# tardis-sn/tardis

Measured on AMD Instinct MI355X. Metric: packets/sec, higher is better.
Workload: dtype f64; 1 GPU; BASELINE configs[2]: 100000000 packets/GPU/step, 20 shells, 500000 lines, macroatom, 0 v-packets, last-interaction tracking on; synthetic opacities (SURVEY 8d, heavy-tailed macro-atom blocks), packets from the device black-body source (T_inner = 10000 K); level_sizes=heavy, packets_per_gpu=100000000, n_shells=20, n_lines=500000, line_interaction_type=macroatom, n_vpackets=0, parallelism=single GPU

## Files before the change

include/tardis_mc.h:

```cpp
#ifndef TARDIS_MC_H
#define TARDIS_MC_H

#include <stdint.h>

#ifdef __cplusplus
extern "C" {
#endif

#define TARDIS_MC_ABI_VERSION 2

enum {
    TARDIS_MC_OK = 0,
    TARDIS_MC_ERR_INVALID_ARGUMENT = -1,
    TARDIS_MC_ERR_HIP = -2,
    TARDIS_MC_ERR_MONTECARLO = -3,
    TARDIS_MC_ERR_MACRO_ATOM = -4,
    TARDIS_MC_ERR_UNSUPPORTED = -5,
    TARDIS_MC_ERR_COMM = -6,
    TARDIS_MC_ERR_STATE = -7
};

enum { TARDIS_MC_LINE_SCATTER = 0, TARDIS_MC_LINE_DOWNBRANCH = 1, TARDIS_MC_LINE_MACROATOM = 2 };

typedef struct TardisMcConfig {
// ... 83 lines not shown
    int64_t dropped;
    int64_t *offsets;
    int64_t *event_id, *interaction_type, *status, *shell_id, *after_shell_id, *line_absorb_id, *line_emit_id;
    double *radius, *before_nu, *before_mu, *before_energy, *after_nu, *after_mu, *after_energy;
} TardisMcEventLog;

typedef struct TardisMcDecomposition {
    int64_t n_classes;
    const int64_t *line_class;
    double time_of_simulation;
    double nu_start, nu_end;
    double *emission;
    double *absorption;
    double *no_interaction;
    double *electron_scatter;
    int64_t *shell_packets;
    int64_t *line_emit_packets;
    int64_t *line_absorb_packets;
    int64_t n_selected, n_line, n_electron_scatter, n_no_interaction;
} TardisMcDecomposition;

typedef struct TardisMcVpacketLog {
    int64_t capacity;
    int64_t count;
    int64_t *offsets;
    int64_t *source_packet;
    double *nus, *energies, *initial_mus, *initial_rs;
    double *last_interaction_in_nu, *last_interaction_in_r;
    int64_t *last_interaction_type, *last_interaction_in_id, *last_interaction_out_id, *last_interaction_shell_id;
} TardisMcVpacketLog;

typedef struct TardisMcContext TardisMcContext;

int tardis_mc_abi_version(void);
int tardis_mc_device_count(void);
int tardis_mc_create(int device_id, TardisMcContext **out_ctx);
void tardis_mc_destroy(TardisMcContext *ctx);
const char *tardis_mc_last_error(const TardisMcContext *ctx);

int tardis_mc_set_option(TardisMcContext *ctx, const char *name, long long value);

int tardis_mc_set_geometry(TardisMcContext *ctx, const TardisMcGeometry *geometry);
int tardis_mc_set_opacity(TardisMcContext *ctx, const TardisMcOpacity *opacity);
int tardis_mc_set_config(TardisMcContext *ctx, const TardisMcConfig *config);
int tardis_mc_set_packets(TardisMcContext *ctx, const TardisMcPackets *packets);
int tardis_mc_reset_estimators(TardisMcContext *ctx);
int tardis_mc_propagate(TardisMcContext *ctx);
int tardis_mc_synchronize(TardisMcContext *ctx);
int tardis_mc_last_propagate_ms(TardisMcContext *ctx, double *out_ms);
int tardis_mc_last_kernel_times(TardisMcContext *ctx, double *out_seed_ms, double *out_propagate_ms, int *out_launches);
int tardis_mc_last_estimator_ms(TardisMcContext *ctx, double *out_ms);
int tardis_mc_last_counters(TardisMcContext *ctx, int64_t out_counters[TARDIS_MC_N_COUNTERS]);
int tardis_mc_last_variant(TardisMcContext *ctx);
int tardis_mc_last_table_offsets(TardisMcContext *ctx);
int tardis_mc_last_compactions(TardisMcContext *ctx);
int tardis_mc_last_tracker_defer(TardisMcContext *ctx);
int tardis_mc_kernel_table_row(int table, int row, int key[12]);
int tardis_mc_last_kernel_key(TardisMcContext *ctx, int *table, int key[12]);
int tardis_mc_progress(TardisMcContext *ctx, int64_t *out_packets_started, int64_t *out_packets_total);
int tardis_mc_get_results(TardisMcContext *ctx, TardisMcResult *result);

int tardis_mc_pcg64_seed(uint64_t seed, uint64_t out_state[4]);
int tardis_mc_create_blackbody_packets(TardisMcContext *ctx, int64_t n_total, int64_t first, int64_t count, double radius,
                                       double temperature, const uint64_t pcg_state[4], uint32_t max_seed_val,
                                       const double *l_array, int64_t n_l);
int tardis_mc_get_packets(TardisMcContext *ctx, double *initial_radii, double *initial_nus, double *initial_mus,
                          double *initial_energies, int64_t *packet_seeds);

int tardis_mc_packet_spectrum(TardisMcContext *ctx, double time_of_simulation, double luminosity_nu_start,
                              double luminosity_nu_end, double *emitted_luminosity_hist, double *reabsorbed_luminosity_hist,
                              double *out_emitted_luminosity, double *out_reabsorbed_luminosity);

int tardis_mc_packet_decomposition(TardisMcContext *ctx, TardisMcDecomposition *d);
int tardis_mc_vpacket_decomposition(TardisMcContext *ctx, TardisMcDecomposition *d);
int tardis_mc_decomposition_path(int64_t n_classes, int64_t n_bins, int64_t n_shells);

int tardis_mc_radiation_field(TardisMcContext *ctx, double time_of_simulation, const double *volume, double w_epsilon,
                              int detailed_optical_window, double *t_radiative, double *dilution_factor, double *j_blues);

int tardis_mc_formal_integral(TardisMcContext *ctx, double inner_temperature, const double *frequencies, int64_t n_frequencies,
                              const double *att_S_ul, const double *Jred_lu, const double *Jblue_lu, int64_t n_impact_parameters,
                              double *luminosity_densities, double *intensities_nu_p);

int tardis_mc_source_function(TardisMcContext *ctx, double time_of_simulation, const double *volume, const double *wavelength_cm,
                              double *att_S_ul, double *Jred_lu, double *Jblue_lu, double *e_dot_u);
int tardis_mc_last_source_iterations(TardisMcContext *ctx);
int tardis_mc_formal_integral_resident(TardisMcContext *ctx, double inner_temperature, const double *frequencies, int64_t n_frequencies,
                                       int64_t n_impact_parameters, double *luminosity_densities, double *intensities_nu_p);

int tardis_mc_formal_integral_interpolated(TardisMcContext *ctx, int64_t interpolate_shells, double inner_temperature,
                                           const double *frequencies, int64_t n_frequencies, int64_t n_impact_parameters,
                                           double *luminosity_densities, double *intensities_nu_p);
int tardis_mc_interpolated_source(TardisMcContext *ctx, int64_t interpolate_shells, double *r_inner_i, double *r_outer_i,
                                  double *electron_density_i, double *tau_sobolev_i, double *att_S_ul_i, double *Jred_lu_i,
                                  double *Jblue_lu_i, double *e_dot_u_i);

typedef struct TardisMcLineData {
    int64_t n_lines;
    int64_t n_transitions;
    int64_t n_levels;
    const double *f_lu;
    const double *wavelength_cm;
    const double *g_lower;
    const double *g_upper;
    const int64_t *level_lower;
    const int64_t *level_upper;
// ... 141 lines not shown
```

tardis_amd/_lib.py:

```python
from __future__ import annotations

import ctypes as C
import os
import subprocess

from . import _abi

_HERE = os.path.dirname(os.path.abspath(__file__))
LIB_PATH = os.environ.get("TARDIS_MC_LIB") or os.path.join(_HERE, "libtardis_mc_hip.so")
_lib = None

_vp, _i, _ll = C.c_void_p, C.c_int, C.c_longlong
SYMBOLS = {
    "tardis_mc_abi_version": (_i, []),
    "tardis_mc_device_count": (_i, []),
    "tardis_mc_create": (_i, [_i, C.POINTER(_vp)]),
    "tardis_mc_destroy": (None, [_vp]),
    "tardis_mc_last_error": (C.c_char_p, [_vp]),
    "tardis_mc_set_option": (_i, [_vp, C.c_char_p, _ll]),
    "tardis_mc_set_geometry": (_i, [_vp, _vp]),
    "tardis_mc_set_opacity": (_i, [_vp, _vp]),
    "tardis_mc_set_config": (_i, [_vp, _vp]),
    "tardis_mc_set_packets": (_i, [_vp, _vp]),
    "tardis_mc_reset_estimators": (_i, [_vp]),
    "tardis_mc_propagate": (_i, [_vp]),
    "tardis_mc_synchronize": (_i, [_vp]),
    "tardis_mc_last_propagate_ms": (_i, [_vp, C.POINTER(C.c_double)]),
    "tardis_mc_last_kernel_times": (_i, [_vp, C.POINTER(C.c_double), C.POINTER(C.c_double), C.POINTER(C.c_int)]),
    "tardis_mc_last_estimator_ms": (_i, [_vp, C.POINTER(C.c_double)]),
    "tardis_mc_last_counters": (_i, [_vp, C.POINTER(C.c_int64)]),
    "tardis_mc_last_variant": (_i, [_vp]),
    "tardis_mc_last_table_offsets": (_i, [_vp]),
    "tardis_mc_last_compactions": (_i, [_vp]),
    "tardis_mc_last_tracker_defer": (_i, [_vp]),
    "tardis_mc_kernel_table_row": (_i, [_i, _i, C.POINTER(_i)]),
    "tardis_mc_last_kernel_key": (_i, [_vp, C.POINTER(_i), C.POINTER(_i)]),
    "tardis_mc_progress": (_i, [_vp, C.POINTER(C.c_int64), C.POINTER(C.c_int64)]),
    "tardis_mc_get_results": (_i, [_vp, _vp]),
    "tardis_mc_pcg64_seed": (_i, [C.c_uint64, C.POINTER(C.c_uint64)]),
    "tardis_mc_create_blackbody_packets": (_i, [_vp, C.c_int64, C.c_int64, C.c_int64, C.c_double, C.c_double,
                                                C.POINTER(C.c_uint64), C.c_uint32, _vp, C.c_int64]),
    "tardis_mc_get_packets": (_i, [_vp] * 6),
    "tardis_mc_packet_spectrum": (_i, [_vp, C.c_double, C.c_double, C.c_double, _vp, _vp, C.POINTER(C.c_double), C.POINTER(C.c_double)]),
    "tardis_mc_packet_decomposition": (_i, [_vp, _vp]),
    "tardis_mc_vpacket_decomposition": (_i, [_vp, _vp]),
    "tardis_mc_decomposition_path": (_i, [C.c_int64, C.c_int64, C.c_int64]),
    "tardis_mc_radiation_field": (_i, [_vp, C.c_double, _vp, C.c_double, C.c_int, _vp, _vp, _vp]),
    "tardis_mc_formal_integral": (_i, [_vp, C.c_double, _vp, C.c_int64, _vp, _vp, _vp, C.c_int64, _vp, _vp]),
    "tardis_mc_source_function": (_i, [_vp, C.c_double, _vp, _vp, _vp, _vp, _vp, _vp]),
    "tardis_mc_last_source_iterations": (_i, [_vp]),
    "tardis_mc_formal_integral_resident": (_i, [_vp, C.c_double, _vp, C.c_int64, C.c_int64, _vp, _vp]),
    "tardis_mc_formal_integral_interpolated": (_i, [_vp, C.c_int64, C.c_double, _vp, C.c_int64, C.c_int64, _vp, _vp]),
    "tardis_mc_interpolated_source": (_i, [_vp, C.c_int64] + [_vp] * 8),
    "tardis_mc_set_line_data": (_i, [_vp, _vp]),
    "tardis_mc_update_opacity": (_i, [_vp, _vp]),
    "tardis_mc_get_opacity": (_i, [_vp] * 6),
    "tardis_mc_last_opacity_update_ms": (_i, [_vp] + [C.POINTER(C.c_double)] * 3),
    "tardis_mc_opacity_update_path": (_i, [C.c_int64]),
    "tardis_mc_set_plasma_data": (_i, [_vp, _vp]),
    "tardis_mc_update_plasma": (_i, [_vp, _vp]),
    "tardis_mc_get_plasma": (_i, [_vp] * 5 + [C.POINTER(C.c_int32)]),
    "tardis_mc_last_plasma_update_ms": (_i, [_vp] + [C.POINTER(C.c_double)] * 4),
    "tardis_mc_plasma_update_path": (_i, [C.c_int64]),
    "tardis_mc_set_ionization_options": (_i, [_vp, _vp]),
    "tardis_mc_check_ionization_options": (_i, [_vp, C.c_int64, _vp, _vp, _vp]),
    "tardis_mc_get_helium": (_i, [_vp, _vp, _vp]),
    "tardis_mc_last_helium_ms": (_i, [_vp, C.POINTER(C.c_double)]),
    "tardis_mc_set_nlte_data": (_i, [_vp, _vp]),
    "tardis_mc_check_nlte_data": (_i, [_vp, C.c_int64, _vp, C.c_int64, _vp, _vp]),
    "tardis_mc_get_nlte": (_i, [_vp, _vp, _vp]),
    "tardis_mc_last_nlte_ms": (_i, [_vp] + [C.POINTER(C.c_double)] * 2),
    "tardis_mc_nlte_solve_path": (_i, [C.c_int64]),
    "tardis_mc_nlte_solve_form": (_i, [C.c_int64]),
    "tardis_mc_set_nlte_collision_data": (_i, [_vp, _vp]),
    "tardis_mc_check_nlte_collision_data": (_i, [_vp, C.c_int64, _vp, C.c_double, C.c_int64, _vp]),
    "tardis_mc_get_nlte_collision_rates": (_i, [_vp, _vp, _vp]),
    "tardis_mc_get_event_log": (_i, [_vp, _vp]),
    "tardis_mc_get_vpacket_log": (_i, [_vp, _vp]),
    "tardis_mc_stream_results": (_i, [_vp, _vp]),
    "tardis_mc_streamed_packets": (_i, [_vp, C.POINTER(C.c_int64), C.POINTER(C.c_int64)]),
    "tardis_mc_run": (_i, [_vp] * 6),
    "tardis_mc_comm_get_unique_id": (_i, [_vp]),
    "tardis_mc_comm_init": (_i, [_vp, _i, _i, _vp]),
    "tardis_mc_allreduce_estimators": (_i, [_vp]),
# ... 40 lines not shown
```

tardis_amd/csrc/propagate_plan.hpp:

```cpp
#pragma once

#include "../../include/tardis_mc.h"

namespace plan {

constexpr int DBG_WALK_LANE_FP64 = 128;
constexpr int DBG_WALK_GROUP_FP64 = 8192;
constexpr int DBG_LONG_INSTANTIATIONS = 1048576;
constexpr int DBG_NO_SCREENING = 33554432;
constexpr int DBG_WAVE_COUNTERS = 1 | 2 | 4 | 16 | 32 | 16384 | 32768 | 65536 | 131072 | 524288 | 2097152 | 4194304 | 8388608 | 16777216 | 134217728 | 268435456;
constexpr int DBG_FP64_WALKS = DBG_WALK_LANE_FP64 | DBG_WALK_GROUP_FP64;
constexpr int DBG_WAVE_CROSS_CHECK = DBG_FP64_WALKS | DBG_LONG_INSTANTIATIONS | DBG_WAVE_COUNTERS;

struct PlanInput {
    int n_shells, n_lines, n_trans;
    long long n_packets;
    long long number_of_vpackets;
    double survival_probability;
    int enable_full_relativity, line_interaction_type;
    bool lines_sorted, prob_negative, have_walk_tables;
    int variant, table_offsets, vpacket_screening;
    long long vpk_wave_min_packets;
    bool track_full;
    int debug_flags;
    bool pfx_valid, pfx_negative;
};

struct Plan {
    int variant;
    bool cooperative;
    bool w64;
    bool screen_on;
    int last_variant, last_table_offsets;
    int error;
    const char *message;
};

inline Plan plan_error(Plan p, const char *message)
{
    p.error = TARDIS_MC_ERR_INVALID_ARGUMENT;
    p.message = message;
    return p;
}

inline Plan plan_propagate(const PlanInput &in)
{
    Plan p{};
    p.error = TARDIS_MC_OK;
    p.message = "";
    const bool vpk = in.number_of_vpackets > 0;
    const bool small_shape = in.n_shells <= 30 && in.n_lines <= 100000;
    const bool screen_auto = (long long)in.n_lines >= 2500LL * (long long)in.n_shells;
    const bool screen = in.vpacket_screening < 0 ? screen_auto : in.vpacket_screening != 0;
    p.screen_on = vpk && in.survival_probability == 0.0 && screen && !(in.debug_flags & DBG_NO_SCREENING) && !(in.pfx_valid && in.pfx_negative);
    const bool prefer_lane_sweeps = !in.enable_full_relativity && !vpk;
    const bool vpk_wave = vpk && (small_shape || (p.screen_on && in.n_packets >= in.vpk_wave_min_packets));
    const int wave_auto = prefer_lane_sweeps ? 3 : 2;
    int variant = in.variant >= 0 ? in.variant : ((vpk && in.number_of_vpackets > 32) ? 0 : (vpk ? (vpk_wave ? 2 : 1) : wave_auto));
    auto is_wave = [](int v) { return v == 2 || v == 3 || v == 4; };
    if (in.prob_negative && (variant == 2 || variant == 3)) variant = 1;
    if (vpk && in.survival_probability > 0.0 && is_wave(variant)) variant = 1;
    if (variant == 4 && !vpk) variant = wave_auto;
    if (in.prob_negative && variant == 4) variant = 1;
    if (in.track_full) {
        const bool wave_ok = in.lines_sorted && !in.prob_negative && !(vpk && (in.number_of_vpackets > 32 || in.survival_probability > 0.0)) &&
                             (in.line_interaction_type == 0 || in.have_walk_tables) && !(in.debug_flags & DBG_WAVE_CROSS_CHECK) && in.n_packets < (1LL << 31);
        variant = (wave_ok && variant != 0) ? 2 : 0;
    }
    bool cooperative = in.lines_sorted && (variant == 1 || is_wave(variant)) && (!vpk || in.number_of_vpackets <= 32);
    const bool big_tables = (long long)in.n_shells * in.n_lines >= (1LL << 28) || (long long)in.n_shells * in.n_trans >= (1LL << 28);
    bool w64 = false;
    if (cooperative && (in.table_offsets == 1 || (in.table_offsets < 0 && big_tables))) {
        if (variant == 4)
            return plan_error(p, "variant 4 (the volley queue) has no 64-bit table offsets: n_shells * n_lines or n_shells * n_trans "
                                 "reaches 2^28, or option table_offsets is 1; use the automatic variant");
        if (is_wave(variant) && (in.debug_flags & DBG_WAVE_CROSS_CHECK))
            return plan_error(p, "the cross-check instantiations of the wave kernel (debug flags 128, 8192, 1048576 and the counter "
                                 "flags) have no 64-bit table offsets");
        if (is_wave(variant) && (long long)in.n_shells * in.n_lines >= (1LL << 32)) {
            if (in.variant >= 0)
                return plan_error(p, "n_shells * n_lines reaches 2^32: the line-visit log of the wave kernels (variants 2-4) "
                                     "indexes (shell, line) in 32 bits; use variant 1 or the automatic variant");
            if (in.track_full) { cooperative = false; variant = 0; }
            else { variant = 1; w64 = true; }
        } else if (is_wave(variant) && in.line_interaction_type != 0 && !in.have_walk_tables) {
            cooperative = false;
            variant = 0;
        } else
            w64 = true;
    }
    if (cooperative && big_tables && !w64)
        return plan_error(p, "n_shells * n_lines or n_shells * n_trans reaches 2^28, the limit of the cooperative kernels' 32-bit "
                             "table offsets, and option table_offsets is 0");
    p.variant = variant;
    p.cooperative = cooperative;
    p.w64 = w64;
    p.last_table_offsets = (w64 || !cooperative) ? 64 : 32;
    p.last_variant = cooperative ? ((variant == 3 && in.enable_full_relativity) ? 2 : variant) : 0;
    if (!cooperative) p.screen_on = false;
    return p;
}

}
```

tardis_amd/csrc/propagate_wave.hpp:

```cpp
#pragma once
#include "mc_device.hpp"
#include "propagate_group.hpp"
#include "estimator_log.hpp"
#include "walk_tables.hpp"
#include "event_log.hpp"
#include "mt_generation.hpp"

namespace mc {

constexpr int WV_STATE_STRIDE = 624;
constexpr int WV_RING = 8, WV_RING_VPK = 16;
enum : int { WS_NEED_PACKET = 0, WS_NEED_TRACE = 1, WS_SWEEP = 2, WS_DONE = 3, WS_WALK = 4, WS_VOLLEY = 5, WS_VCARRY = 6 };
constexpr int RES_PENDING = -1;
constexpr int WV_DBG_FLAGS = 1 | 2 | 4 | 16 | 32 | 16384 | 32768 | 65536 | 131072 | 524288 | 2097152 | 4194304 | 8388608 | 16777216 | 134217728 | 268435456;
constexpr int WV_RESERVE = 32;

struct WaveShared {
    double nu[64], rcp_nu[64], comov_nu[64], chi[64], rcp_chi[64], tau_event[64], d_cont0[64];
    double d_boundary[64];
    int res_info[64], res_line[64];
    unsigned rng_a[64], rng_b[64];
    int cursor[64], rowfast[64];
    int queue[64];
};
constexpr size_t WAVE_SHARED_LS_BYTES = sizeof(WaveShared) - 3 * 64 * sizeof(int);
static_assert(offsetof(WaveShared, queue) + sizeof(int) * 64 == sizeof(WaveShared) && offsetof(WaveShared, cursor) + 3 * 64 * sizeof(int) == sizeof(WaveShared),
              "cursor | rowfast | queue are the last 768 bytes: the lane-sweep instantiations leave them out, the pooled volleys' item list lies over them");
struct WaveSharedFull {
    double r[64], mu[64];
};

template <bool FULL, bool VPK, bool LS = false, bool SL = false>
__host__ __device__ constexpr size_t wave_kernel_lds_bytes(int n_shells)
{
    return (LS ? WAVE_SHARED_LS_BYTES : sizeof(WaveShared)) + (FULL ? sizeof(WaveSharedFull) : 0) + (size_t)(VPK ? WV_RING_VPK : WV_RING) * 64 * sizeof(double) +
           (size_t)(VPK ? 6 : 5) * (size_t)n_shells * sizeof(double) +
           (SL ? (size_t)n_shells * 2 * sizeof(unsigned) : 0);
}

struct __attribute__((aligned(16))) VpResult {
    double nu, energy, mu0;
    int used, visits, err, pad;
};
struct __attribute__((aligned(16))) VpPark {
    double r, mu, nu, energy, tau, mu0, rcp_nu, margin, v0_r, v0_energy;
    int shell, next_line, owner, item, q, used, avail, head, v0_shell, v0_line;
    unsigned visits;
    int flags;
};
constexpr int VP_ROUND = 6;
static_assert(2 * VP_ROUND + 3 <= 16, "a round's mu and roulette draws, plus the 4 doubles of the refill that completes them, must fit WV_RING_VPK");

struct __attribute__((aligned(16))) VolleyRequest {
    double r, mu, nu, energy;
    int shell, next_line, vdone, cnt;
    unsigned pred_bits;
    int pad0, pad1, pad2;
    double draws[WV_RING_VPK];
};
// ... 5 lines not shown
    double t_exp;
    const int2 *line_block;
    int ls_min_active, ls_max_steps;
    int walk_min_active;
    int vq_min_active;
};
struct LaunchRec;
struct __attribute__((aligned(16))) LaneSave {
    double r, mu, nu, energy, dop;
    double s_tau, s_tau_event, s_kp, s_xb;
    double d_cont0, d_boundary;
    double ring[WV_RING_VPK];
    int shell, next_line, status, state, pkt, pflags, r_gpos, r_head, r_cnt;
    int trk_count, trk_boundary, flags;
    int s_line;
    unsigned s_row;
    int res_info, res_line, pre_blk_x, pre_blk_y;
    unsigned rng_a, rng_b;
    int vseq;
    unsigned pred_bits;
    int vdone, pad_v0, pad_v1, pad_v2;
    double walk_inv_new, walk_block, trk_nu, trk_mu, trk_energy;
    double walk_event, pad_w;
};
struct WaveSave {
    long long res_next, res_end;
    int exhausted, done;
    int log_chunk, log_gen;
    unsigned long long cnt[7];
};
struct WaveCold {
    GroupArgs P;
    DeviceProblem D;
    EstimatorLog log;
    uint32_t *seeded_states;
    long long chunk_first, chunk_count;
    const LaunchRec *launch;
    VpResult *vp_scratch;
    VpPark *vp_park;
    int vp_carry_min_active;
    int trk_defer;
    LaneSave *save;
    WaveSave *wsave;
    int resume;
    int drain_split;
    unsigned *suspended;
    VolleyRequest *vq_req;
    unsigned *vq_items;
    unsigned *vq_count;
    int log_continue;
    int log_gen;
    double *vq_jsave;
    int rng_complete;
};

__global__ void __launch_bounds__(64) late_list_kernel(const LaneSave *__restrict__ save, const WaveSave *__restrict__ wsave, int waves, long long first, long long end,
                                                       unsigned *__restrict__ late, unsigned *__restrict__ late_count, unsigned capacity)
{
    const int w = blockIdx.x, lane = threadIdx.x;
    if (w >= waves) return;
    const WaveSave ws = wsave[w];
    if (ws.done) return;
    const LaneSave &v = save[(size_t)w * 64 + lane];
    const bool live = v.state != WS_NEED_PACKET && v.state != WS_DONE && (long long)v.pkt >= first && (long long)v.pkt < end;
    const long long r0 = ws.res_next > first ? ws.res_next : first, r1 = ws.res_end < end ? ws.res_end : end;
    const int n_res = r1 > r0 ? (int)(r1 - r0) : 0;
    const unsigned long long lm = __ballot(live);
    const unsigned n_live = (unsigned)__popcll(lm);
    unsigned base = 0;
    if (lane == 0 && n_live + (unsigned)n_res > 0) base = atomicAdd(late_count, n_live + (unsigned)n_res);
    base = (unsigned)__shfl((int)base, 0);
    if (live) {
        const unsigned pos = base + (unsigned)__popcll(lm & ((1ull << lane) - 1ull));
        if (pos < capacity) late[pos] = (unsigned)v.pkt;
    }
    for (int k = lane; k < n_res; k += 64) {
        const unsigned pos = base + n_live + (unsigned)k;
        if (pos < capacity) late[pos] = (unsigned)(r0 + k);
    }
}

__global__ void __launch_bounds__(64) drain_census_kernel(const LaneSave *__restrict__ save, const WaveSave *__restrict__ wsave, int waves, long long n_packets,
                                                          unsigned *__restrict__ out)
{
    const int w = blockIdx.x, lane = threadIdx.x;
    if (w >= waves) return;
    const WaveSave ws = wsave[w];
    if (ws.done) return;
    const int state = save[(size_t)w * 64 + lane].state;
    const unsigned n_live = (unsigned)__popcll(__ballot(state != WS_NEED_PACKET && state != WS_DONE));
    const unsigned n_need = (unsigned)__popcll(__ballot(state == WS_NEED_PACKET));
    const long long r1 = ws.res_end < n_packets ? ws.res_end : n_packets;
    if (lane == 0) {
        if (n_live) atomicAdd(out, n_live);
        if (r1 > ws.res_next) atomicAdd(out + 1, (unsigned)(r1 - ws.res_next));
        atomicAdd(out + 2, 1u);
        if (n_need) atomicAdd(out + 3, n_need);
    }
}
__global__ void __launch_bounds__(64) drain_compact_kernel(const LaneSave *__restrict__ save, const WaveSave *__restrict__ wsave, const uint32_t *__restrict__ states, int waves,
                                                           LaneSave *__restrict__ dst_save, uint32_t *__restrict__ dst_states, unsigned *__restrict__ counter, unsigned density)
{
    const int w = blockIdx.x, lane = threadIdx.x;
    if (w >= waves) return;
    const WaveSave ws = wsave[w];
    if (ws.done) return;
// ... 90 lines not shown
            }
            s.owner = -1;
        } else {
            const int n_in = min(G, L - s.cur0);
            visits += (unsigned long long)n_in;
            s.tau_carry = gbcast<G>(tau_incl, n_in - 1);
            s.d_cont_carry = exact_div<FAST>(s.tau_event - s.tau_carry, s.chi, s.rcp_chi);
            s.cur0 += G;
            s.nu_line = nu_next;
            s.tau_line = tau_next;
        }
    } else {
        if (j == 0) {
            const bool cont = s.d_cont_carry < s.d_boundary;
            sh.d_boundary[s.owner] = cont ? s.d_cont_carry : s.d_boundary;
            sh.res_line[s.owner] = 0;
            sh.res_info[s.owner] = (cont ? 2 : 1) | 8;
        }
        s.owner = -1;
    }
}


__device__ __forceinline__ int lane_exact_line(const WaveHot &P, int line, double nu_line, double tau_line, double tau_prev, double nu,
                                               double comov_nu, double chi, double tau_event, double d_boundary, double &distance)
{
    const double tau_incl = tau_prev + tau_line;
    const double d_cont = (tau_event - tau_prev) / chi;
    const bool is_last = line == P.n_lines - 1;
    const double nu_diff = comov_nu - nu_line;
    const double q = nu_diff / nu;
    const bool close = fabs(q) < CLOSE_LINE_THRESHOLD;
    const bool err = !is_last && !close && !(nu_diff >= 0);
    const double d_far = q * C_LIGHT * P.t_exp;
    const double d_trace = is_last ? MISS_DISTANCE : (close ? 0.0 : d_far);
    const double tau_combined = tau_incl + chi * d_trace;
    double dmin = d_trace;
    if (d_boundary < dmin) dmin = d_boundary;
    if (d_cont < dmin) dmin = d_cont;
    const bool stop_b = !err && d_trace != 0 && dmin == d_boundary;
    const bool stop_e = !err && d_trace != 0 && !stop_b && dmin == d_cont;
    const bool stop_l = !err && !stop_b && !stop_e && tau_combined > tau_event && !P.disable_line_scattering;
    distance = stop_b ? d_boundary : (stop_e ? d_cont : d_trace);
    return stop_b ? 1 : (stop_e ? 2 : (stop_l ? 3 : (err ? 4 : 0)));
}
constexpr int LS_CHUNK = 8;
#ifndef TMC_STRAIGHT_A
#define TMC_STRAIGHT_A 0
#endif
#ifndef TMC_LS_CHUNK_NT
#define TMC_LS_CHUNK_NT 10
#endif
constexpr int LS_CHUNK_NT = TMC_LS_CHUNK_NT;

__global__ void __launch_bounds__(256) macro_cumulative_kernel(const double *__restrict__ prob_t, double *__restrict__ cum_t,
                                                                const int *__restrict__ block_edge, int n_blocks, long long n_trans,
                                                                int n_shells, int *negative)
{
    const long long i = (long long)blockIdx.x * blockDim.x + threadIdx.x;
    if (i >= (long long)n_blocks * n_shells) return;
    const int b = (int)(i % n_blocks), s = (int)(i / n_blocks);
    const double *p = prob_t + (long long)s * n_trans;
    double *c = cum_t + (long long)s * n_trans;
    double carry = 0.0;
    bool neg = false;
    const int b0 = block_edge[b], b1 = block_edge[b + 1];
    for (int k0 = b0; k0 < b1; k0 += 8) {
        double v[8];
#pragma unroll
        for (int q = 0; q < 8; ++q) v[q] = k0 + q < b1 ? p[k0 + q] : 0.0;
#pragma unroll
        for (int q = 0; q < 8; ++q)
            if (k0 + q < b1) {
                neg |= !(v[q] >= 0.0);
                carry += v[q];
                c[k0 + q] = carry;
            }
    }
    if (neg) atomicOr(negative, 1);
}

struct __attribute__((aligned(16))) TrackerRecord {
    double before_nu, before_mu, before_energy, radius, after_mu;
    int shell, type, absorb, emit, count, valid;
};
static_assert(sizeof(TrackerRecord) == 64, "TrackerRecord is one 64-byte request");

__global__ void __launch_bounds__(256) tracker_unpack_kernel(DeviceProblem D, long long first, long long count, const unsigned *__restrict__ index = nullptr)
{
    const long long j = (long long)blockIdx.x * blockDim.x + threadIdx.x;
    if (j >= count) return;
    const long long i = index ? (long long)index[j] : first + j;
    const double e = D.out_e[i];
    if (e == -99.0) return;
    const TrackerRecord r = reinterpret_cast<const TrackerRecord *>(D.li_rec)[i];
    const bool any = r.valid != 0 && r.count > 0;
    const double nan = __builtin_nan("");
    const double nu = D.out_nu[i], en = fabs(e);
    D.li_radius[i] = any ? r.radius : nan;
    D.li_nu[i] = any ? nu : nan; D.li_energy[i] = any ? en : nan;
    D.li_before_nu[i] = any ? r.before_nu : nan; D.li_before_mu[i] = any ? r.before_mu : nan; D.li_before_energy[i] = any ? r.before_energy : nan;
    D.li_after_nu[i] = any ? nu : nan; D.li_after_mu[i] = any ? r.after_mu : nan; D.li_after_energy[i] = any ? en : nan;
    D.li_shell_id[i] = any ? r.shell : -1; D.li_interaction_type[i] = any ? r.type : -1;
    D.li_line_absorb_id[i] = any ? r.absorb : -1; D.li_line_emit_id[i] = any ? r.emit : -1;
    D.li_interactions_count[i] = any ? r.count : 0;
}
// ... 234 lines not shown
            for (int i = 0; i < 4; ++i) sw[i] = d_boundary <= d_line_of(min(w0 + i, L - 1), wn[i]);
            int hit = -1;
            if (sw[0]) { if (w0 == start + 1) hit = 0; }
            else if (sw[1]) hit = 1;
            else if (sw[2]) hit = 2;
            else if (sw[3]) hit = 3;
            if (hit >= 0 && w0 + hit <= L - 1) {
                e = w0 + hit;
                double pe = wp[0];
#pragma unroll
                for (int i = 1; i < 4; ++i) if (hit == i) pe = wp[i];
                seg = pe - p_start;
            } else {
                if (hit >= 0) e = L - 1;
                else e = vp_walk_to_stop(nu_line_g, L, start, w0, sw[0], [&](int k, double nl) { return d_boundary <= d_line_of(k, nl); });
                seg = prow[(unsigned)min(e, L)] - p_start;
            }
        }
        n_sum = min(e, L) - start;
        vvisits += (unsigned)((e < L) ? (e - start + 1) : (L - start));
        v.next_line = e;
    }
    const double tau_shell = tau_cont + seg;
    v.tau += tau_shell;
    margin += 2.3e-16 * (geo[3 * S + v.shell] + (double)(n_sum + 4) * tau_shell + 2.0 * v.tau);
    cross_shell(v.shell, status, delta, S);
    if (v.tau - 2.0 * margin > P.tau_russian) {
        if (draws_left <= 0) return ERR_UNSUPPORTED;
        --draws_left;
        const double ev = draw();
        if (!(ev > P.survival_probability)) return 2;
        v.energy = 0.0;
        return 1;
    }
    if (!(v.tau + 2.0 * margin < P.tau_russian)) return 2;
    if (status == ST_EMITTED) return 2;
    const double new_r = sqrt(v.r * v.r + d_boundary * d_boundary + 2.0 * v.r * d_boundary * v.mu);
    v.mu = (v.mu * v.r + d_boundary) / new_r;
    v.r = new_r;
    return 0;
}

template <bool FULL, bool TRACK, int G, bool VPK, bool LS = false, bool XWALK = true, int WPE = (VPK ? 3 : 4), int NT = 0, bool SL = false,
          bool FT = false, bool WIDE = false, bool VLI = false>
__global__ void __launch_bounds__(64) __attribute__((amdgpu_waves_per_eu(WPE, WPE))) propagate_wave_kernel(WaveHot H, const WaveCold *__restrict__ W)
{
    static_assert(!WIDE || (!XWALK && NT == 0 && !SL), "64-bit row offsets: the compact walks, the separate line and tau tables, the log by bin");
    static_assert(!FT || TRACK, "the full tracking counts rows with the last-interaction tracker's counters");
    static_assert(NT == 0 || (LS && !VPK && !FULL), "the interleaved sweep table is read by the lane sweeps only");
    static_assert(!SL || !VPK, "the shell-sorted log is built for the instantiations without v-packets");
    static_assert(NT != 2 || WPE != 3, "aligned runs are eight lines long");
    constexpr bool DEFER = TRACK && LS && !VPK && !FT && !XWALK;
    constexpr bool RNGC = LS && !VPK;
    extern __shared__ __attribute__((aligned(16))) unsigned char lds_raw[];
    WaveShared &sh = *reinterpret_cast<WaveShared *>(lds_raw);
    constexpr size_t SH_BYTES = LS ? WAVE_SHARED_LS_BYTES : sizeof(WaveShared);
    WaveSharedFull &shf = *reinterpret_cast<WaveSharedFull *>(lds_raw + SH_BYTES);
    constexpr int RING = VPK ? WV_RING_VPK : WV_RING;
    double *ring = reinterpret_cast<double *>(lds_raw + SH_BYTES + (FULL ? sizeof(WaveSharedFull) : 0));
    double *lds_J = ring + RING * 64;
    double *lds_nubar = lds_J + H.n_shells;
    double *lds_geo = lds_nubar + H.n_shells;
    int *lds_lchunk = reinterpret_cast<int *>(lds_geo + (VPK ? 4 : 3) * H.n_shells);
    unsigned *lds_lused = reinterpret_cast<unsigned *>(lds_lchunk + H.n_shells);
    if (SL)
        for (int s = threadIdx.x; s < H.n_shells; s += 64) { lds_lchunk[s] = -1; lds_lused[s] = 0u; }
    for (int s = threadIdx.x; s < H.n_shells; s += 64) {
        lds_geo[s] = glob(W->P.r_inner)[s]; lds_geo[H.n_shells + s] = glob(W->P.r_outer)[s]; lds_geo[2 * H.n_shells + s] = glob(W->P.n_e)[s];
        if (VPK) lds_geo[3 * H.n_shells + s] = W->P.tau_rowsum ? glob(W->P.tau_rowsum)[s] : 0.0;
    }
    const int lane = threadIdx.x;
    {
        const double *js = (W->resume && W->vq_jsave) ? W->vq_jsave + (size_t)blockIdx.x * (size_t)(2 * H.n_shells) : nullptr;
        for (int s = lane; s < 2 * H.n_shells; s += 64) lds_J[s] = js ? glob(js)[s] : 0.0;
    }

    const int j = lane & (G - 1);
    const int group_lane0 = lane & ~(G - 1);
    const double t = H.t_exp;
    const int L = H.n_lines;

    Packet p;
    p.r = p.mu = p.nu = p.energy = 0.0; p.shell = 0; p.next_line_id = 0; p.status = ST_IN_PROCESS;
    int state = WS_NEED_PACKET;
    int pkt = 0;
    double dop = 1.0;
    int pflags = 0;
    int r_gpos = 0, r_head = 0, r_cnt = 0;
    unsigned draws = 0, events = 0, macro = 0;
    unsigned long long vvisits_total = 0;
    unsigned vcount = 0;
    int vseq = 0;
    unsigned pred_bits = 0;
    unsigned long long vtraced_total = 0;
    int vq_done = 0;
    bool v_out = false;
    bool v_parked = false;
    bool vq_fresh = false;
    int trk_count = 0, trk_boundary = 0;
    bool trk_any = false;
    int ev_chunk = -1;
    unsigned ev_used = 0;
    bool ev_row = false;
    int ev_type = 0, ev_shell = 0, ev_after = 0, ev_absorb = -1, ev_emit = -1;
    double ev_bnu = 0.0, ev_bmu = 0.0, ev_be = 0.0;
    bool exhausted = false;
// ... 152 lines not shown
        double *const jb = P.jblue_t, *const ed = P.edot_t;
        bool log_full = false;
        if (SL && log.region_capacity > 0 && __ballot(state != WS_DONE) != 0ull) {
            bool need = false;
            if (lane < H.n_shells) need = lds_lchunk[lane] < 0 || lds_lused[lane] + 64u > log.region_capacity;
            if (__ballot(need)) {
                bool full = false;
                if (need) {
                    if (lds_lchunk[lane] >= 0) glob(log.region_count)[lds_lchunk[lane]] = min(lds_lused[lane], log.region_capacity);
                    const unsigned c = gatomic_add_u32(log.pool_next, 1u);
                    full = c >= (unsigned)log.n_regions;
                    lds_lchunk[lane] = full ? -1 : (int)c;
                    lds_lused[lane] = 0u;
                }
                log_full = __ballot(full) != 0ull && W->save != nullptr;
            }
        }
        if (!SL && log.region_capacity > 0 && (log_chunk < 0 || log_used + 64 > log.region_capacity) && __ballot(state != WS_DONE) != 0ull) {
            if (lane == 0 && log_chunk >= 0) glob(log.region_count)[log_chunk] = min(log_used, log.region_capacity);
            unsigned c = 0;
            if (lane == 0) c = gatomic_add_u32(log.pool_next, 1u);
            c = (unsigned)__builtin_amdgcn_readfirstlane((int)c);
            log_used = 0;
            if (c < (unsigned)log.n_regions) log_chunk = (int)c;
            else { log_chunk = -1; log_full = W->save != nullptr; }
        }
        bool vq_stop = false;
        if (VPK && W->vq_items) {
            const unsigned long long waiting = __ballot(state == WS_VOLLEY && vq_fresh);
            const unsigned long long can = __ballot(state != WS_DONE && !(state == WS_VOLLEY && vq_fresh));
            vq_stop = waiting != 0ull && __popcll(can) <= H.vq_min_active;
        }
        const int drain_live = W->drain_split ? __popcll(__ballot(state != WS_DONE)) : 0;
        const bool drain_stop = W->drain_split && W->save && exhausted && res_next == res_end && logged_any && drain_live != 0 && drain_live <= W->drain_split;
        if (log_full || vq_stop || drain_stop) {
            suspended_log = log_full;
            suspended_drain = drain_stop && !log_full && !vq_stop;
            MC_G LaneSave &v = *glob(W->save + ((size_t)blockIdx.x * 64 + lane));
            v.r = p.r; v.mu = p.mu; v.nu = p.nu; v.energy = p.energy; v.dop = dop;
            v.s_tau = s_tau; v.s_tau_event = s_tau_event; v.s_kp = s_kp; v.s_xb = s_xb;
            v.d_cont0 = sh.d_cont0[lane]; v.d_boundary = sh.d_boundary[lane];
#pragma unroll
            for (int q = 0; q < WV_RING_VPK; ++q) v.ring[q] = q < RING ? ring[q * 64 + lane] : 0.0;
            v.shell = p.shell; v.next_line = p.next_line_id; v.status = p.status; v.state = state; v.pkt = pkt; v.pflags = pflags;
            v.r_gpos = r_gpos; v.r_head = r_head; v.r_cnt = r_cnt;
            v.trk_count = trk_count; v.trk_boundary = trk_boundary;
            v.flags = (trk_any ? 1 : 0) | (s_active ? 2 : 0) | (s_fast ? 4 : 0);
            v.s_line = s_line; v.s_row = (unsigned)s_row;
            v.res_info = sh.res_info[lane]; v.res_line = sh.res_line[lane]; v.pre_blk_x = pre_blk.x; v.pre_blk_y = pre_blk.y;
            v.rng_a = sh.rng_a[lane]; v.rng_b = sh.rng_b[lane];
            v.vseq = vseq; v.pred_bits = pred_bits; v.vdone = vq_done; v.pad_v0 = v.pad_v1 = v.pad_v2 = 0;
            v.walk_inv_new = sh.chi[lane]; v.walk_block = sh.rcp_chi[lane]; v.walk_event = sh.tau_event[lane]; v.pad_w = 0.0;
            v.trk_nu = sh.nu[lane]; v.trk_mu = sh.rcp_nu[lane]; v.trk_energy = sh.comov_nu[lane];
            suspended = true;
            break;
        }
        if constexpr (RNGC) {
            const unsigned long long todo = W->rng_complete ? __ballot(state != WS_NEED_PACKET && state != WS_DONE && (r_gpos >> 16) == 1) : 0ull;
            if (todo) {
                mtg::mt_complete_generations_wave<WV_STATE_STRIDE>(glob(seeded_states) + (size_t)blockIdx.x * 64 * WV_STATE_STRIDE, todo, r_gpos & 0x3ff, lane);
                __builtin_amdgcn_fence(__ATOMIC_SEQ_CST, "workgroup");
                if ((todo >> lane) & 1ull) r_gpos |= 0x20000;
            }
        }
        const bool ready = state == WS_SWEEP && !(LS && s_active);
        refill(__ballot((ready || state == WS_NEED_TRACE || state == WS_WALK) && r_cnt <= RING - 4), seeded_states);
        int err = 0, type = 0, emit = -1, mb0 = 0, mb1 = 0;
        double inv_new = 1.0, distance = 0.0, emit_nu_walk = 0.0;
        bool in_macro = false, interacted = false;
        bool want_volley = false;
        const bool resumed = state == WS_WALK;
        if (resumed) {
            in_macro = true; interacted = true; type = IT_LINE;
            inv_new = sh.chi[lane];
            const int2 blk = reinterpret_cast<const int2 *>(sh.rcp_chi)[lane];
            mb0 = blk.x; mb1 = blk.y;
        }
        {
            int n_visit = 0, start = 0;
            if (ready) {
                const int info = sh.res_info[lane];
                distance = sh.d_boundary[lane];
                const int code = info & 7;
                start = p.next_line_id;
                const int stop_line = (info & 8) ? L : sh.res_line[lane];
                n_visit = stop_line - start + ((code == 3) ? 1 : 0);
                if (LS) visits += (unsigned long long)(unsigned)(stop_line - start + ((info & 8) ? 0 : 1));
                if (!(info & 8)) p.next_line_id = stop_line;
                if (code == 4) err = ERR_MONTECARLO;
                type = code == 1 ? IT_BOUNDARY : (code == 2 ? IT_ESCATTERING : IT_LINE);
                if (DBG && (P.debug_flags & 1)) n_visit = 0;
            }
            const unsigned long long have = __ballot(n_visit > 0);
            if (have) {
                unsigned my = 0;
                int my_chunk = log_chunk;
                if (SL) {
                    logged_any = true;
                    if (n_visit > 0) { my = atomicAdd(&lds_lused[p.shell], 1u); my_chunk = lds_lchunk[p.shell]; }
                } else {
                    my = log_used + (unsigned)__popcll(have & ((1ull << lane) - 1ull));
                    log_used += (unsigned)__popcll(have);
                    logged_any = true;
                }
                if (n_visit > 0) {
                    LineVisitRecord rec;
// ... 714 lines not shown
                    if (state == WS_VCARRY) state = WS_NEED_TRACE;
                    if (verr || vdone == n_v) in_volley = false;
                }
                if (cut && !__ballot(in_volley && !v_out)) break;
            }
            if (in_volley && v_out) {
                state = WS_VCARRY;
                vq_done = vdone;
            }
            if (tracing) {
                VpPark k;
                k.r = vs.r; k.mu = vs.mu; k.nu = vs.nu; k.energy = vs.energy; k.tau = vs.tau; k.mu0 = vs.mu0; k.shell = vs.shell; k.next_line = vs.next_line;
                k.rcp_nu = v_rcp_nu; k.margin = v_margin; k.v0_r = v0_r; k.v0_energy = v0_energy; k.v0_shell = v0_shell; k.v0_line = v0_line;
                k.owner = w_owner; k.item = w_item; k.q = w_q; k.used = w_used; k.avail = w_avail; k.head = w_head;
                k.visits = my_visits; k.flags = (v_fast ? 1 : 0) | (screening ? 2 : 0);
                gstore(W->vp_park + ((size_t)blockIdx.x * 64 + lane), k);
                v_parked = true;
            }
            }
            if (verr) {
                const long long i = chunk_first + pkt;
                gatomic_min_i64(&C->first_error[0], i);
                glob(C->out_nu)[i] = (double)verr;
                glob(C->out_e)[i] = -99.0;
                state = WS_NEED_PACKET;
            }
        }
        TMC_SEC(4)
        refill(__ballot(state == WS_NEED_TRACE && r_cnt < 1), seeded_states);
        {
            const bool go = state == WS_NEED_TRACE;
            if (go) {
                const double velocity = p.r / t;
                dop = doppler_factor<FULL>(velocity, p.mu);
                double chi_e = lds_geo[2 * P.n_shells + p.shell] * P.sigma_thomson;
                if (FULL) chi_e *= dop;
                double d_boundary;
                int delta;
                distance_boundary(p.r, p.mu, lds_geo[p.shell], lds_geo[P.n_shells + p.shell], d_boundary, delta);
                const double tau_event = -mcm::log(draw());
                const double comov_nu = p.nu * dop;
                ++events;
                const bool fast = mid_range(p.nu) && mid_range(chi_e) && mid_range(tau_event) && mid_range(p.energy) &&
                                  mid_range(p.r) && mid_range(comov_nu) && mid_range(P.t_exp) && !(DBG && (P.debug_flags & 4));
                pflags = (fast ? 1 : 0) | ((delta + 1) << 1);
                if (LS) {
                    sh.d_cont0[lane] = chi_e; sh.d_boundary[lane] = d_boundary;
                    s_tau_event = tau_event;
                    s_tau = 0.0; s_line = p.next_line_id; s_row = NT != 0 ? (row_t<WIDE>)((unsigned)p.shell * P.nt_stride) : row_of<WIDE>(p.shell, L);
                    s_kp = ((chi_e * P.tc) / p.nu) * (1.0 + 0x1p-40);
                    s_xb = ((d_boundary * p.nu) * P.rcp_tc) * (1.0 - 0x1p-40);
                    s_fast = fast && mid_range(s_kp);
                    s_active = true;
                } else {
                    sh.nu[lane] = p.nu; sh.rcp_nu[lane] = 1.0 / p.nu; sh.comov_nu[lane] = comov_nu;
                    sh.chi[lane] = chi_e; sh.rcp_chi[lane] = 1.0 / chi_e;
                    sh.tau_event[lane] = tau_event; sh.d_boundary[lane] = d_boundary;
                    sh.d_cont0[lane] = tau_event / chi_e;
                    if (FULL) { shf.r[lane] = p.r; shf.mu[lane] = p.mu; }
                    sh.cursor[lane] = p.next_line_id;
                    sh.rowfast[lane] = (int)((WIDE ? (unsigned)p.shell : (unsigned)p.shell * (unsigned)L) | (fast ? 0x80000000u : 0u));
                }
                state = WS_SWEEP;
            }
            if (!LS) {
                const unsigned long long go_mask = __ballot(go);
                if (go) sh.queue[(q_tail + __popcll(go_mask & ((1ull << lane) - 1ull))) & 63] = lane;
                q_tail += __popcll(go_mask);
            }
        }

        TMC_SEC(5)
        if (LS) {
            const int ls_cut = (DBG && (H.debug_flags & 16777216)) ? H.ls_min_active : (H.ls_min_active * __popcll(__ballot(state != WS_DONE))) >> 6;
            for (int step = 0;; ++step) {
                const unsigned long long act = __ballot(s_active);
                if (!act) break;
                if (step > 0) {
                    const unsigned long long waiting = __ballot(state == WS_SWEEP && !s_active);
                    if (waiting && (__popcll(act) <= ls_cut || step >= H.ls_max_steps)) break;
                }
                if (DBG) ++dbg_rounds;
                if (s_active) {
                    const double *__restrict__ pn = H.nu_line + (unsigned)s_line;
                    const double *__restrict__ pt = H.tau_t + (s_row + (unsigned)s_line);
                    constexpr int CH = (WPE == 3 && !VPK) ? 12 : ((NT == 1 && WPE == 4) ? LS_CHUNK_NT : LS_CHUNK);
                    double nl[CH], tl[CH];
                    typedef double nt2 __attribute__((ext_vector_type(2)));
                    const unsigned nt_at = s_row + (unsigned)s_line;
                    const nt2 *__restrict__ pq = reinterpret_cast<const nt2 *>(H.tau_t) + (NT == 2 ? (nt_at & ~7u) : nt_at);
                    const int k0 = NT == 2 ? (int)(nt_at & 7u) : 0;
                    if constexpr (NT != 0) {
#pragma unroll
                        for (int k = 0; k < CH; ++k) { const nt2 e = pq[k]; nl[k] = e.x; tl[k] = e.y; }
                    } else {
#pragma unroll
                        for (int k = 0; k < CH; ++k) { nl[k] = pn[k]; tl[k] = pt[k]; }
                    }
                    if (DBG && (H.debug_flags & 524288)) {
                        const unsigned touch = reinterpret_cast<const unsigned *>(pt + min(2 * LS_CHUNK - 1, L - 1 + LS_CHUNK - s_line))[1];
                        if (touch == 0x7ff00001u) ++dbg_rounds;
                    }
                    int adv = 0;
                    const double comov = p.nu * dop;
                    const int n_fast = L - 1 - s_line;
                    bool alive;
                    double f_nu, f_tau;
                    if constexpr ((WPE == 3 && !VPK) || (TMC_STRAIGHT_A != 0 && WPE == 4 && NT == 1)) {
                        double t[CH + 1];
                        t[0] = s_tau;
#pragma unroll
                        for (int k = 0; k < CH; ++k) t[k + 1] = t[k] + tl[k];
                        unsigned fail = 0;
#pragma unroll
                        for (int k = CH - 1; k >= 0; --k) {
                            const double X = comov - nl[k];
                            const double x = s_kp * X;
                            const double sum = t[k + 1] + x;
                            bool ok;
                            if constexpr (NT != 0) ok = (k > 0 || X >= 0.0) && X < s_xb && sum < s_tau_event;
                            else {
                                const double D = s_tau_event - t[k];
                                ok = X >= 0.0 && X < s_xb && x < D && sum <= s_tau_event;
                            }
                            fail = fail + fail + (ok ? 0u : 1u);
                        }
                        if constexpr (NT != 0) fail |= s_fast ? (1u << CH) : 1u;
                        else fail |= 1u << (s_fast ? min(max(n_fast, 0), CH) : 0);
                        adv = __builtin_ctz(fail);
                        alive = adv == CH;
                        double ts = t[0];
#pragma unroll
                        for (int k = 1; k <= CH; ++k)
                            if (adv >= k) ts = t[k];
                        s_tau = ts;
                        if constexpr (NT != 0) { const nt2 e = pq[alive ? 0 : adv]; f_nu = e.x; f_tau = e.y; }
                        else { f_nu = pn[alive ? 0 : adv]; f_tau = pt[alive ? 0 : adv]; }
                    } else {
                        alive = s_fast;
                        f_nu = nl[0]; f_tau = tl[0];
                        if constexpr (NT == 2) {
#pragma unroll
                            for (int k = 1; k < CH; ++k)
                                if (k == k0) { f_nu = nl[k]; f_tau = tl[k]; }
                        }
                        int kf = alive ? CH : k0;
#pragma unroll
                        for (int k = 0; k < CH; ++k) {
                            if (alive && (NT != 2 || k >= k0)) {
                                const double X = comov - nl[k];
                                const double x = s_kp * X;
                                const double tau_n = s_tau + tl[k];
                                const double sum = tau_n + x;
                                bool ok;
                                if constexpr (NT != 0) {
                                    ok = (k > (NT == 2 ? k0 : 0) || X >= 0.0) && X < s_xb && sum < s_tau_event;
                                } else {
                                    const double D = s_tau_event - s_tau;
                                    ok = k - k0 < n_fast && X >= 0.0 && X < s_xb && x < D && sum <= s_tau_event;
                                }
                                if (ok) s_tau = tau_n;
                                else { alive = false; kf = k; f_nu = nl[k]; f_tau = tl[k]; }
                            }
                        }
                        adv = kf - k0;
                    }
                    if (!alive) {
                        const double chi = sh.d_cont0[lane], d_bound = sh.d_boundary[lane];
                        const int line = s_line + adv;
                        int code;
                        double dist;
                        if (line < L) {
                            code = lane_exact_line(H, line, f_nu, f_tau, s_tau, p.nu, comov, chi, s_tau_event, d_bound, dist);
                            if (!code) { s_tau = s_tau + f_tau; ++adv; }
                        } else {
                            const double d_cont = (s_tau_event - s_tau) / chi;
                            const bool cont = d_cont < d_bound;
                            dist = cont ? d_cont : d_bound;
                            code = (cont ? 2 : 1) | 8;
                        }
                        if (code) {
                            sh.d_boundary[lane] = dist; sh.res_info[lane] = code; sh.res_line[lane] = (code & 8) ? 0 : line;
                            if (code == 3 && H.line_block) pre_blk = H.line_block[(unsigned)line];
                            s_active = false;
                        }
                    }
                    s_line += adv;
                }
            }
            TMC_SEC(6)
            continue;
        }

        SweepSlot<WIDE> cur;
        cur.owner = -1; cur.cur0 = 0; cur.row = 0; cur.fast = true;
        cur.nu = cur.rcp_nu = cur.comov_nu = cur.chi = cur.rcp_chi = cur.tau_event = cur.d_boundary = cur.r = cur.mu = 0.0;
        cur.tau_carry = cur.d_cont_carry = cur.nu_line = cur.tau_line = 0.0;
        int nxt_owner = -1, n_cursor = 0;
        unsigned n_rowfast = 0;
        double n_nu = 0.0, n_tau = 0.0;
        for (;;) {
            const int avail = q_tail - q_head;
            const unsigned long long busy = __ballot(cur.owner >= 0 || nxt_owner >= 0);
            if (avail == 0 && !busy) break;
            __builtin_amdgcn_s_waitcnt(0x0F70);
            if (DBG) ++dbg_rounds;
            if (cur.owner < 0 && nxt_owner >= 0) {
                const int o = nxt_owner;
                cur.owner = o;
                nxt_owner = -1;
                cur.nu = sh.nu[o]; cur.rcp_nu = sh.rcp_nu[o]; cur.comov_nu = sh.comov_nu[o];
                cur.chi = sh.chi[o]; cur.rcp_chi = sh.rcp_chi[o]; cur.tau_event = sh.tau_event[o]; cur.d_boundary = sh.d_boundary[o];
                if (FULL) { cur.r = shf.r[o]; cur.mu = shf.mu[o]; }
                cur.fast = (n_rowfast >> 31) != 0;
                cur.cur0 = n_cursor; cur.row = WIDE ? row_of<WIDE>((int)(n_rowfast & 0x7fffffffu), L) : (row_t<WIDE>)(n_rowfast & 0x7fffffffu);
                cur.nu_line = n_nu; cur.tau_line = n_tau;
                cur.tau_carry = 0.0;
                cur.d_cont_carry = sh.d_cont0[o];
            }
            {
                const unsigned long long free_groups = __ballot(nxt_owner < 0 && j == 0);
                if (avail > 0 && free_groups) {
                    const int rank = __popcll(free_groups & ((1ull << group_lane0) - 1ull));
                    if (nxt_owner < 0 && rank < avail) {
                        nxt_owner = sh.queue[(q_head + rank) & 63];
                        n_cursor = sh.cursor[nxt_owner];
                        n_rowfast = (unsigned)sh.rowfast[nxt_owner];
                        const int line = n_cursor + j;
                        const bool in = line < L;
                        n_nu = in ? H.nu_line[(unsigned)line] : 0.0;
                        const row_t<WIDE> n_row = WIDE ? row_of<WIDE>((int)(n_rowfast & 0x7fffffffu), L) : (row_t<WIDE>)(n_rowfast & 0x7fffffffu);
                        n_tau = in ? H.tau_t[n_row + (unsigned)line] : 0.0;
// ... 214 lines not shown
```

tardis_amd/csrc/tardis_mc_hip.hip:

```cpp
#include <hip/hip_runtime.h>
#include <dlfcn.h>

#include <algorithm>
#include <chrono>
#include <cstdarg>
#include <cstdio>
#include <cmath>
#include <cstring>
#include <functional>
#include <numeric>
#include <atomic>
#include <mutex>
#include <string>
#include <vector>

#include "../../include/tardis_mc.h"
#include "mc_device.hpp"
#include "propagate_lane.hpp"
#include "event_log.hpp"
#include "propagate_group.hpp"
#include "estimator_log.hpp"
#include "estimator_partition.hpp"
#include "propagate_wave.hpp"
#include "packet_source.hpp"
#include "formal_integral.hpp"
#include "formal_interpolate.hpp"
#include "source_function.hpp"
#include "tau_prefix.hpp"
#include "propagate_plan.hpp"
#include "packet_decomposition.hpp"
#include "decomposition_plan.hpp"
#include "vpacket_log.hpp"
#include "opacity_update.hpp"
#include "opacity_update_plan.hpp"
#include "plasma_update.hpp"
#include "plasma_update_plan.hpp"
#include "nlte_excitation.hpp"
#include "nlte_plan.hpp"

static_assert(plan::DBG_WAVE_COUNTERS == mc::WV_DBG_FLAGS, "propagate_plan.hpp repeats the wave kernel's list of counter flags");

namespace {

thread_local std::string g_create_error;

struct DevBuf {
    void *p = nullptr;
    size_t cap = 0;
    hipError_t ensure(size_t bytes)
    {
        if (bytes <= cap && p) return hipSuccess;
        if (p) { hipError_t e = hipFree(p); p = nullptr; cap = 0; if (e != hipSuccess) return e; }
        size_t want = bytes ? bytes : 16;
        hipError_t e = hipMalloc(&p, want);
        if (e == hipSuccess) cap = want;
        return e;
    }
    void release() { if (p) { (void)hipFree(p); p = nullptr; cap = 0; } }
    template <typename T> T *as() const { return static_cast<T *>(p); }
};
struct ScopedDevBuf : DevBuf {
    ScopedDevBuf() = default;
    ScopedDevBuf(const ScopedDevBuf &) = delete;
    ScopedDevBuf &operator=(const ScopedDevBuf &) = delete;
    ~ScopedDevBuf() { release(); }
};
void release_buffer(DevBuf &b) { b.release(); }
template <size_t N> void release_buffer(DevBuf (&bufs)[N])
{
    for (DevBuf &b : bufs) b.release();
}
template <typename... Bufs> void release_buffers(Bufs &...bufs) { (release_buffer(bufs), ...); }
void destroy_event(hipEvent_t &e)
{
    if (e) { (void)hipEventDestroy(e); e = nullptr; }
}
template <size_t N> void destroy_events(hipEvent_t (&ev)[N])
{
    for (hipEvent_t &e : ev) destroy_event(e);
}
void destroy_events(std::vector<hipEvent_t> &ev)
// ... 70 lines not shown
    int variant = -1;
    int blocks_per_cu = 16;
    int debug_flags = 0;
    int group_size = 0;
    long long vpk_wave_min_packets = 100000;
    int vpk_wide_registers = 1;
    int last_variant = -1;
    int table_offsets = -1;
    int last_table_offsets = -1;
    int waves_per_simd = 4;
    int last_kernel_table = -1;
    int last_kernel_key[12] = {};
    void release()
    {
        release_buffers(r_inner, r_outer, grid, staging, rng_state, counters, first_error, next_packet, problem_dev);
        destroy_event(ev_start); destroy_event(ev_stop); destroy_events(ev_chunk);
        destroy_stream(stream);
    }
    struct OpacityTables {
        DevBuf nu_line, tau_t, n_e, prob_t, cum_t, trans_nu, line2level, block_edge, ttype, dest, tline, line_block, trans_rec, bucket_first;
        int bucket_shift = 0, bucket_n = 0;
        int bucket_lines_permille = 750;
        long long bucket_kmin = 0;
        bool lines_sorted = true;
        bool prob_negative = false;
        std::vector<int> h_idx[5];
        std::vector<double> h_nu;
        bool h_macro = false;
        void release() { release_buffers(nu_line, tau_t, n_e, prob_t, cum_t, trans_nu, line2level, block_edge, ttype, dest, tline, line_block, trans_rec, bucket_first); }
    } ot;
    struct WalkTables {
        DevBuf cum16, rec16, quad_info, line_block_c;
        DevBuf hot_sec, hot_mass, hot_flag, blk_tab;
        bool have_hot = false;
        long long n_hot_blocks = 0;
        int walk_hot = -1;
        int walk_hot_min_mass = 800, walk_hot_min_mass_long = 400;
        unsigned cum16_stride = 0;
        bool have_walk_tables = false;
        int walk_sector_packing = 1;
        void release() { release_buffers(cum16, rec16, quad_info, line_block_c, hot_sec, hot_mass, hot_flag, blk_tab); }
    } wt;
    struct ScreeningTables {
        DevBuf tau_pfx, tau_rowsum, pfx_flag;
        bool pfx_valid = false, pfx_negative = false;
        int vpacket_screening = -1;
        void release() { release_buffers(tau_pfx, tau_rowsum, pfx_flag); }
    } sc;
    struct SweepTable {
        int sweep_table = -1;
        DevBuf nt_t;
        bool nt_valid = false, nt_negative = false;
        unsigned nt_stride = 0;
        void release() { release_buffers(nt_t); }
    } sw;
    struct Estimators {
        DevBuf est;
        size_t est_S = 0, est_L = 0, est_G = 0;
        int est_copies = 1;
        bool est_valid = false;
        bool est_propagated = false;
        void release() { release_buffers(est); }
    } es;
    struct Packets {
        long long n_packets = 0;
        DevBuf r0, mu0, nu0, e0, seeds, out_nu, out_e;
        DevBuf li_f64[9], li_i64[5], li_rec;
        bool track = true;
        bool li_valid = false;
        DevBuf dc_work;
        void release() { release_buffers(r0, mu0, nu0, e0, seeds, out_nu, out_e, li_f64, li_i64, li_rec, dc_work); }
    } pk;
    struct VpacketLog {
        DevBuf vlog_count, vlog_packet, vlog_seq, vlog_nu, vlog_energy, vlog_mu, vlog_r;
        long long vlog_capacity = 0;
        bool vlog_capacity_user = false;
        bool vlog_li = false;
        DevBuf vl_counts, vl_offsets, vl_tiles, vl_cols, vl_errors;
        bool vl_valid = false;
        bool vl_li = false;
        bool vl_consolidated = false;
        long long vl_packets = 0, vl_capacity = 0, vl_count = 0;
        void release() { release_buffers(vlog_count, vlog_packet, vlog_seq, vlog_nu, vlog_energy, vlog_mu, vlog_r, vl_counts, vl_offsets, vl_tiles, vl_cols, vl_errors); }
    } vl;
    struct EventLog {
        bool track_full = false;
        long long evlog_capacity = 0;
        long long evlog_max_bytes = 16LL << 30;
        DevBuf ev_rows, ev_fill, ev_state, ev_counts, ev_offsets, ev_tiles, ev_cols;
        bool ev_valid = false;
        long long ev_packets = 0, ev_capacity = 0, ev_slots = 0;
        unsigned ev_chunk_rows = 128, ev_n_chunks = 0;
        void release() { release_buffers(ev_rows, ev_fill, ev_state, ev_counts, ev_offsets, ev_tiles, ev_cols); }
    } el;
    struct WaveResources {
        bool walk_min_active_user = false, ls_min_active_user = false;
        int walk_min_active = 8;
        int tracker_defer = 1, last_tracker_defer = -1;
        int rng_complete = 1;
        long long tracker_pack_max_lines = 0;
        int ls_min_active = 8, ls_max_steps = 1 << 30;
        int drain_split = 0;
        int log_tail_packets = 8;
        int log_tail_split = 1;
        int est_accumulate = 3;
        int est_pipeline = 1;
        DevBuf log_part;
// ... 149 lines not shown
    int rank = 0, world = 1;
};

namespace {

int fail(TardisMcContext *ctx, int code, const char *fmt, ...)
{
    char buf[512];
    va_list ap;
    va_start(ap, fmt);
    vsnprintf(buf, sizeof buf, fmt, ap);
    va_end(ap);
    if (ctx) ctx->err = buf; else g_create_error = buf;
    return code;
}

#define HIP_TRY(ctx, expr)                                                                                      \
    do {                                                                                                        \
        hipError_t _e = (expr);                                                                                 \
        if (_e != hipSuccess)                                                                                   \
            return fail(ctx, TARDIS_MC_ERR_HIP, "%s failed: %s (%s:%d)", #expr, hipGetErrorString(_e), __FILE__, \
                        __LINE__);                                                                              \
    } while (0)

__global__ void transpose_kernel(const double *__restrict__ in, double *__restrict__ out, long long rows, long long cols)
{
    __shared__ double tile[32][33];
    long long bx = (long long)blockIdx.x * 32, by = (long long)blockIdx.y * 32;
    for (int j = threadIdx.y; j < 32; j += 8) {
        long long r = by + j, c = bx + threadIdx.x;
        if (r < rows && c < cols) tile[j][threadIdx.x] = in[r * cols + c];
    }
    __syncthreads();
    for (int j = threadIdx.y; j < 32; j += 8) {
        long long c = bx + j, r = by + threadIdx.x;
        if (r < rows && c < cols) out[c * rows + r] = tile[threadIdx.x][j];
    }
}

__global__ void __launch_bounds__(256) interleave_kernel(const double *__restrict__ nu_line, const double *__restrict__ tau_t, double2 *__restrict__ nt,
                                                         long long L, long long S, long long stride, long long total, int *negative)
{
    bool neg = false;
    for (long long i = (long long)blockIdx.x * blockDim.x + threadIdx.x; i < total; i += (long long)gridDim.x * blockDim.x) {
        const long long s = i / stride, l = i - s * stride;
        const bool in = s < S && l < L;
        const double tau = in ? tau_t[s * L + l] : 0.0;
        neg |= !(tau >= 0.0);
        nt[i] = make_double2((in && l < L - 1) ? nu_line[l] : -__builtin_inf(), tau);
    }
    if (neg) atomicOr(negative, 1);
}

template <typename T>
__global__ void store_value_kernel(T *dst, const T v)
{
    if (threadIdx.x == 0 && blockIdx.x == 0) *dst = v;
}
template <typename T>
hipError_t store_value(hipStream_t st, T *dst, const T &v)
{
    static_assert(sizeof(T) <= 3584, "argument block too large for the kernel-argument buffer");
    hipLaunchKernelGGL(store_value_kernel<T>, dim3(1), dim3(64), 0, st, dst, v);
    return hipGetLastError();
}
struct FirstErrorInit { long long v[2]; };

__global__ void reduce_copies_kernel(double *base, long long n, long long stride, int copies)
{
    long long i = (long long)blockIdx.x * blockDim.x + threadIdx.x;
    long long step = (long long)gridDim.x * blockDim.x;
    for (; i < n; i += step) {
        double s = base[i];
        for (int c = 1; c < copies; ++c) { s += base[i + c * stride]; base[i + c * stride] = 0.0; }
        base[i] = s;
    }
}

__global__ void debug_eval_kernel(int op, const double *x, const double *y, double *out, long long n, uint32_t *scratch)
{
    long long i = (long long)blockIdx.x * blockDim.x + threadIdx.x;
    if (op == 7) {
        if (i == 0) {
            mc::Rng rng;
            rng.seed(scratch, (uint32_t)x[0]);
            for (long long k = 0; k < n; ++k) out[k] = rng.random();
        }
        return;
    }
    if (i >= n) return;
    double a = x[i], b = y ? y[i] : 0.0, r;
    switch (op) {
    case 0: r = a + b; break;
    case 1: r = a * b; break;
    case 2: r = a / b; break;
    case 3: r = sqrt(a); break;
    case 4: r = mcm::log(a); break;
    case 5: r = mcm::exp(a); break;
    case 6: r = a * b + a; break;
    case 8: r = floor(a); break;
    case 9: r = ((mc::mid_range(a) || a == 0.0) && mc::mid_range(b)) ? mc::exact_div<true>(a, b, 1.0 / b) : a / b; break;
    default: r = 0.0;
    }
    out[i] = r;
}

// ... 233 lines not shown
template <size_t N>
int ensure_events(TardisMcContext *ctx, hipEvent_t (&ev)[N])
{
    for (hipEvent_t &e : ev)
        if (!e) HIP_TRY(ctx, hipEventCreate(&e));
    return TARDIS_MC_OK;
}
int event_intervals_ms(TardisMcContext *ctx, const hipEvent_t *ev, int n, double *const *out)
{
    HIP_TRY(ctx, hipEventSynchronize(ev[n]));
    for (int k = 0; k < n; ++k) {
        float ms = 0.f;
        HIP_TRY(ctx, hipEventElapsedTime(&ms, ev[k], ev[k + 1]));
        if (out[k]) *out[k] = ms;
    }
    return TARDIS_MC_OK;
}

constexpr double H_PLANCK = 6.62606957e-27, K_BOLTZMANN = 1.3806488e-16, M_ELECTRON = 9.10938291e-28;

enum Rung { RUNG_LINE_DATA, RUNG_PLASMA_DATA, RUNG_NLTE_DATA, RUNG_COLLISION_DATA };
void drop_from(TardisMcContext *ctx, Rung rung)
{
    switch (rung) {
    case RUNG_LINE_DATA: ctx->ou.have = ctx->ou.valid = false; [[fallthrough]];
    case RUNG_PLASMA_DATA: ctx->pl.have = ctx->pl.valid = false; ctx->he.have = ctx->he.valid = false; [[fallthrough]];
    case RUNG_NLTE_DATA: ctx->nl.have = ctx->nl.valid = false; [[fallthrough]];
    case RUNG_COLLISION_DATA: ctx->nc.have = ctx->nc.valid = false;
    }
}

enum Cause {
    GEOMETRY_REPLACED,
    OPACITY_TOPOLOGY_REPLACED,
    OPACITY_UPDATE_BEGINS,
    OPACITY_VALUES_REPLACED,
    ESTIMATORS_CHANGED,
    CONFIG_REPLACED,
    PACKETS_REPLACED,
    PROPAGATE_BEGINS
};
void drop_products(TardisMcContext *ctx, Cause cause)
{
    switch (cause) {
    case GEOMETRY_REPLACED:
    case OPACITY_UPDATE_BEGINS:
    case ESTIMATORS_CHANGED: ctx->sf.valid = false; break;
    case OPACITY_TOPOLOGY_REPLACED: ctx->sf.valid = ctx->sf.topo_valid = ctx->sf.exp_valid = false; break;
    case OPACITY_VALUES_REPLACED:
        ctx->sf.valid = ctx->sf.exp_valid = false;
        ctx->wt.have_walk_tables = ctx->wt.have_hot = false;
        ctx->sc.pfx_valid = false;
        ctx->sw.nt_valid = false;
        break;
    case CONFIG_REPLACED: ctx->vl.vl_valid = ctx->vl.vl_consolidated = false; break;
    case PACKETS_REPLACED:
        ctx->pk.li_valid = false;
        ctx->vl.vl_valid = ctx->vl.vl_consolidated = false;
        break;
    case PROPAGATE_BEGINS:
        ctx->el.ev_valid = ctx->pk.li_valid = ctx->sf.valid = ctx->rs.valid = false;
        ctx->vl.vl_valid = ctx->vl.vl_consolidated = false;
        break;
    }
}

void per_packet_device_arrays(TardisMcContext *ctx, void *dev[16])
{
    dev[0] = ctx->pk.out_nu.p; dev[1] = ctx->pk.out_e.p;
    for (int k = 0; k < 9; ++k) dev[2 + k] = ctx->pk.track ? ctx->pk.li_f64[k].p : nullptr;
    for (int k = 0; k < 5; ++k) dev[11 + k] = ctx->pk.track ? ctx->pk.li_i64[k].p : nullptr;
}
void per_packet_host_arrays(const TardisMcResult *r, void *host[16])
{
    host[0] = r->output_nus; host[1] = r->output_energies;
    double *f[] = {r->li_radius, r->li_nu, r->li_energy, r->li_before_nu, r->li_before_mu, r->li_before_energy, r->li_after_nu, r->li_after_mu, r->li_after_energy};
    for (int k = 0; k < 9; ++k) host[2 + k] = f[k];
    int64_t *g[] = {r->li_shell_id, r->li_interaction_type, r->li_line_absorb_id, r->li_line_emit_id, r->li_interactions_count};
    for (int k = 0; k < 5; ++k) host[11 + k] = g[k];
}

__global__ void __launch_bounds__(256) narrow_seeds_kernel(const long long *__restrict__ in, long long n, uint32_t *__restrict__ out)
{
    const long long i = (long long)blockIdx.x * blockDim.x + threadIdx.x;
    if (i < n) out[i] = (uint32_t)in[i];
}

bool vlog_li_call(const TardisMcContext *ctx)
{
    return ctx->vl.vlog_li && ctx->cfg.enable_vpacket_tracking && ctx->cfg.number_of_vpackets > 0 && ctx->vl.vlog_capacity > 0;
}

mc::DeviceProblem make_device_problem(TardisMcContext *ctx)
{
    mc::DeviceProblem P{};
    P.n_packets = ctx->pk.n_packets;
    P.r0 = ctx->pk.r0.as<double>(); P.mu0 = ctx->pk.mu0.as<double>(); P.nu0 = ctx->pk.nu0.as<double>(); P.e0 = ctx->pk.e0.as<double>();
    P.seeds = ctx->pk.seeds.as<uint32_t>();
    P.out_nu = ctx->pk.out_nu.as<double>(); P.out_e = ctx->pk.out_e.as<double>();
    if (ctx->pk.track) {
        double **f[] = {&P.li_radius, &P.li_nu, &P.li_energy, &P.li_before_nu, &P.li_before_mu, &P.li_before_energy,
                        &P.li_after_nu, &P.li_after_mu, &P.li_after_energy};
        for (int k = 0; k < 9; ++k) *f[k] = ctx->pk.li_f64[k].as<double>();
        long long **g[] = {&P.li_shell_id, &P.li_interaction_type, &P.li_line_absorb_id, &P.li_line_emit_id,
                           &P.li_interactions_count};
        for (int k = 0; k < 5; ++k) *g[k] = ctx->pk.li_i64[k].as<long long>();
// ... 227 lines not shown
    P.evlog.dropped = ctx->el.ev_state.as<unsigned long long>() + 1;
    P.evlog.counts = ctx->el.ev_counts.as<int>();
    P.evlog.chunk_rows = ctx->el.ev_chunk_rows;
    P.evlog.n_chunks = (unsigned)chunks;
    ctx->el.ev_packets = n;
    ctx->el.ev_capacity = cap;
    ctx->el.ev_slots = slots;
    ctx->el.ev_n_chunks = (unsigned)chunks;
    return TARDIS_MC_OK;
}

struct PropagateCall {
    plan::Plan plan;
    int cus;
    bool vpk, full;
    bool rs_armed;
    int tune_pending;
    int tune_slot;
};

plan::PlanInput plan_input(const TardisMcContext *ctx)
{
    const TardisMcConfig &c = ctx->cfg;
    plan::PlanInput in{};
    in.n_shells = ctx->n_shells; in.n_lines = ctx->n_lines; in.n_trans = ctx->n_trans; in.n_packets = ctx->pk.n_packets;
    in.number_of_vpackets = c.number_of_vpackets; in.survival_probability = c.survival_probability;
    in.enable_full_relativity = c.enable_full_relativity; in.line_interaction_type = c.line_interaction_type;
    in.lines_sorted = ctx->ot.lines_sorted; in.prob_negative = ctx->ot.prob_negative; in.have_walk_tables = ctx->wt.have_walk_tables;
    in.variant = ctx->variant; in.table_offsets = ctx->table_offsets; in.vpacket_screening = ctx->sc.vpacket_screening;
    in.vpk_wave_min_packets = ctx->vpk_wave_min_packets; in.track_full = ctx->el.track_full; in.debug_flags = ctx->debug_flags;
    in.pfx_valid = ctx->sc.pfx_valid; in.pfx_negative = ctx->sc.pfx_negative;
    return in;
}

int build_screening_tables(TardisMcContext *ctx)
{
    if (ctx->sc.pfx_valid) return TARDIS_MC_OK;
    const size_t S = (size_t)ctx->n_shells, L = (size_t)ctx->n_lines;
    HIP_TRY(ctx, ctx->sc.tau_pfx.ensure((S * (L + 1) + 8) * sizeof(double)));
    HIP_TRY(ctx, ctx->sc.tau_rowsum.ensure(S * sizeof(double)));
    HIP_TRY(ctx, ctx->sc.pfx_flag.ensure(sizeof(int)));
    HIP_TRY(ctx, hipMemsetAsync(ctx->sc.pfx_flag.p, 0, sizeof(int), ctx->stream));
    hipLaunchKernelGGL(mc::tau_prefix_kernel, dim3((unsigned)S), dim3(256), 0, ctx->stream, ctx->ot.tau_t.as<double>(), (int)L,
                       ctx->sc.tau_pfx.as<double>(), ctx->sc.tau_rowsum.as<double>(), ctx->sc.pfx_flag.as<int>());
    HIP_TRY(ctx, hipGetLastError());
    int neg = 0;
    HIP_TRY(ctx, hipMemcpyAsync(&neg, ctx->sc.pfx_flag.p, sizeof(int), hipMemcpyDeviceToHost, ctx->stream));
    HIP_TRY(ctx, hipStreamSynchronize(ctx->stream));
    ctx->sc.pfx_negative = neg != 0;
    ctx->sc.pfx_valid = true;
    return TARDIS_MC_OK;
}

int build_sweep_table(TardisMcContext *ctx)
{
    const unsigned long long stride = ((unsigned long long)ctx->n_lines + 7ull) & ~7ull;
    if (ctx->sw.nt_valid || stride * (unsigned long long)ctx->n_shells + 32ull >= (1ull << 28)) return TARDIS_MC_OK;
    const long long total = (long long)(stride * (unsigned long long)ctx->n_shells) + 32;
    HIP_TRY(ctx, ctx->sw.nt_t.ensure((size_t)total * 16));
    HIP_TRY(ctx, ctx->sc.pfx_flag.ensure(sizeof(int)));
    HIP_TRY(ctx, hipMemsetAsync(ctx->sc.pfx_flag.p, 0, sizeof(int), ctx->stream));
    hipLaunchKernelGGL(interleave_kernel, dim3((unsigned)std::min<long long>((total + 255) / 256, 65536)), dim3(256), 0, ctx->stream, ctx->ot.nu_line.as<double>(),
                       ctx->ot.tau_t.as<double>(), ctx->sw.nt_t.as<double2>(), (long long)ctx->n_lines, (long long)ctx->n_shells, (long long)stride, total,
                       ctx->sc.pfx_flag.as<int>());
    HIP_TRY(ctx, hipGetLastError());
    int neg = 0;
    HIP_TRY(ctx, hipMemcpyAsync(&neg, ctx->sc.pfx_flag.p, sizeof(int), hipMemcpyDeviceToHost, ctx->stream));
    HIP_TRY(ctx, hipStreamSynchronize(ctx->stream));
    ctx->sw.nt_negative = neg != 0;
    ctx->sw.nt_stride = (unsigned)stride;
    ctx->sw.nt_valid = true;
    return TARDIS_MC_OK;
}

int lane_sweep_tuner(TardisMcContext *ctx, PropagateCall &call, bool *ls3)
{
    auto &tn = ctx->lt.ls_tune;
    const bool w64 = call.plan.w64;
    const int mode = ctx->cfg.line_interaction_type;
    *ls3 = false;
    const bool all_drain = ctx->pk.n_packets < 4LL * 64 * 16 * call.cus;
    if (ctx->lt.ls_waves_per_simd == 3 || (ctx->lt.ls_waves_per_simd == 0 && all_drain)) *ls3 = true;
    else if (ctx->lt.ls_waves_per_simd == 0 && ctx->wv.pass_cus == 0) {
        if (tn.n != ctx->pk.n_packets || tn.lines != ctx->n_lines || tn.shells != ctx->n_shells || tn.mode != mode || tn.table != ctx->sw.sweep_table || tn.wide != (int)w64) {
            tn.n = ctx->pk.n_packets; tn.lines = ctx->n_lines; tn.shells = ctx->n_shells; tn.mode = mode; tn.table = ctx->sw.sweep_table;
            tn.wide = (int)w64;
            tn.phase = 0; tn.choice = 0;
            tn.ms[0][0] = tn.ms[0][1] = tn.ms[1][0] = tn.ms[1][1] = -1.0;
        } else if (call.tune_pending >= 0) {
            float ms = 0.f;
            HIP_TRY(ctx, hipEventSynchronize(ctx->lt.ev_tune[1]));
            HIP_TRY(ctx, hipEventElapsedTime(&ms, ctx->lt.ev_tune[0], ctx->lt.ev_tune[1]));
            tn.ms[call.tune_pending >> 1][call.tune_pending & 1] = ms;
        } else if (tn.phase >= 2 && tn.phase <= 5)
            tn.phase -= 1;
        if (tn.phase == 0) *ls3 = false;
        else if (tn.phase <= 4) { *ls3 = (tn.phase & 1) == 0; call.tune_slot = 2 * (*ls3 ? 1 : 0) + ((tn.phase - 1) >> 1); }
        else {
            if (tn.phase == 5) {
                const bool all = tn.ms[0][0] > 0.0 && tn.ms[0][1] > 0.0 && tn.ms[1][0] > 0.0 && tn.ms[1][1] > 0.0;
                tn.choice = (all && std::min(tn.ms[1][0], tn.ms[1][1]) < 0.97 * std::min(tn.ms[0][0], tn.ms[0][1])) ? 1 : 0;
            }
            *ls3 = tn.choice == 1;
        }
        if (tn.phase < 6) ++tn.phase;
        if (call.tune_slot >= 0)
            for (int k = 0; k < 2; ++k)
                if (!ctx->lt.ev_tune[k]) HIP_TRY(ctx, hipEventCreate(&ctx->lt.ev_tune[k]));
    }
    return TARDIS_MC_OK;
}

struct WaveChoice {
    WaveKernelKey key;
    WaveKernelFn fn;
    size_t lds;
    int waves_per_cu;
    int max_waves_per_cu;
    bool compact_walk, ls3;
    int tiles, n_bins;
    bool partition;
};

int choose_wave_kernel(TardisMcContext *ctx, PropagateCall &call, mc::GroupArgs &P, WaveChoice &w)
{
    const TardisMcConfig &c = ctx->cfg;
    const bool vpk = call.vpk, full = call.full, w64 = call.plan.w64, vq = call.plan.variant == 4;
    WaveKernelKey &k = w.key;
    k = WaveKernelKey{};
    k.full = full; k.track = ctx->pk.track; k.vpk = vpk;
    k.lane_sweep = call.plan.variant == 3 && !full;
    k.waves_per_simd = vpk ? 3 : 4;
    if (wave_kernel_lds(k, ctx->n_shells) > 64 * 1024) return fail(ctx, TARDIS_MC_ERR_INVALID_ARGUMENT, "n_shells too large for the LDS J/nu_bar accumulator");
    w.waves_per_cu = std::max(1, std::min(ctx->waves_per_simd > 0 ? 4 * ctx->waves_per_simd : 16, (int)((160 * 1024) / wave_kernel_lds(k, ctx->n_shells))));
    w.compact_walk = c.line_interaction_type != 0 && ctx->wt.have_walk_tables && !(ctx->debug_flags & plan::DBG_FP64_WALKS);
    k.xwalk = (c.line_interaction_type != 0 && !w.compact_walk) || (ctx->debug_flags & (plan::DBG_LONG_INSTANTIATIONS | plan::DBG_WAVE_COUNTERS)) != 0;
    if (w64 && k.xwalk) return fail(ctx, TARDIS_MC_ERR_INVALID_ARGUMENT, "the fp64 macro-atom walks have no 64-bit table offsets");
    const int GW = ctx->group_size ? ctx->group_size : (ctx->n_lines <= 100000 ? 8 : 16);
    k.width = k.lane_sweep ? 16 : GW;
    if (vpk && !k.xwalk && !w64 && !ctx->el.track_full && (k.lane_sweep || GW == 16 || GW == 8) &&
        ((ctx->vpk_wide_registers == 1 && w.waves_per_cu <= 8) || ctx->vpk_wide_registers == 2))
        k.waves_per_simd = 2;
    w.ls3 = false;
    if (k.lane_sweep && !vpk && !k.xwalk) {
        int rc = lane_sweep_tuner(ctx, call, &w.ls3);
        if (rc) return rc;
        if (w.ls3) k.waves_per_simd = 3;
        if (!w64 && ctx->sw.sweep_table != 0) {
            rc = build_sweep_table(ctx);
            if (rc) return rc;
            if (ctx->sw.nt_valid && !ctx->sw.nt_negative) {
                k.nt = (ctx->sw.sweep_table == 2 && !w.ls3) ? 2 : 1;
                P.nt_t = ctx->sw.nt_t.as<double>(); P.nt_stride = ctx->sw.nt_stride;
            }
        }
    }
    w.max_waves_per_cu = k.waves_per_simd == 2 ? 8 : (w.ls3 ? 12 : 16);
    w.tiles = std::max((ctx->n_lines + mc::EST_TILE - 1) / mc::EST_TILE, 1);
    w.n_bins = ctx->n_shells * w.tiles;
    w.partition = ctx->wv.est_pipeline == 1 && w.tiles <= mc::PART_LOCAL_BUCKETS && ctx->n_shells <= mc::PART_LOCAL_BUCKETS;
    k.shell_log = k.lane_sweep && !vpk && !k.xwalk && !w64 && !vq && w.partition && ctx->wv.log_by_shell != 0 && ctx->n_shells <= 64 &&
                  ((!w.ls3 && k.nt == 1) || (w.ls3 && k.nt == 0));
    if (ctx->el.track_full) {
        k.full_tracking = true; k.track = true; k.width = 16;
    }
    if (w64) { k.wide = true; if (k.width == 4) k.width = 8; }
    k.vli = vlog_li_call(ctx);
    w.fn = find_kernel(WAVE_KERNELS, k);
    if (!w.fn)
        return fail(ctx, TARDIS_MC_ERR_STATE, "propagate: no such instantiation of the wave kernel: FULL, TRACK, G, VPK, LS, XWALK, WPE, NT, SL, FT, WIDE, VLI = %s",
                    key_text(k).c_str());
    record_kernel(ctx, 2, k);
    w.lds = wave_kernel_lds(k, ctx->n_shells);
    return TARDIS_MC_OK;
}

struct LogMemory { bool known; double avail, total; };
LogMemory log_memory(const TardisMcContext *ctx)
{
    size_t free_b = 0, total_b = 0;
    if (hipMemGetInfo(&free_b, &total_b) != hipSuccess) return LogMemory{false, 0.0, 0.0};
    const double have = (double)(ctx->wv.log_records[0].cap + ctx->wv.log_records[1].cap + ctx->wv.log_keys[0].cap + ctx->wv.log_keys[1].cap +
                                 ctx->wv.log_sorted[0].cap + ctx->wv.log_sorted[1].cap + ctx->wv.log_part.cap);
    return LogMemory{true, (double)free_b + have, (double)total_b};
}
constexpr double LOG_RECORD_BYTES = (double)(sizeof(mc::LineVisitRecord) + sizeof(unsigned));
double log_bytes_per_record(int sets, bool partition)
{
    return partition ? sets * LOG_RECORD_BYTES + (double)sizeof(mc::LineVisitRecord) : sets * (LOG_RECORD_BYTES + (double)sizeof(unsigned));
}
constexpr double LOG_MEMORY_SHARE = 0.6;

struct LogSizing {
    bool one_set;
    int n_sets;
    unsigned region_capacity;
    unsigned long long n_chunks;
    size_t set_records;
    double tail_records;
    bool tail_plan, tail_possible, want_split, want_compact, set1_inside;
};

int size_line_log(TardisMcContext *ctx, const PropagateCall &call, const WaveChoice &w, long long n, int waves, bool cu_split, LogSizing &s)
{
    const bool vpk = call.vpk, vq = call.plan.variant == 4, partition = w.partition, shell_log = w.key.shell_log;
    long long log_capacity = ctx->wv.log_capacity;
    s.one_set = ctx->wv.log_sets == 1;
    if (ctx->wv.log_sets == 0 && partition && !vq && !vpk && ctx->wv.drain_split == 0 && ctx->wv.drain_compact == 0 && ctx->wv.epoch_split == 0 && ctx->wv.pass_cus == 0) {
        double two_set_capacity = (double)ctx->wv.log_capacity;
        if (!ctx->wv.log_capacity_user) {
            const LogMemory m = log_memory(ctx);
            if (m.known) two_set_capacity = std::min(two_set_capacity, LOG_MEMORY_SHARE * m.avail / log_bytes_per_record(2, true));
        }
        const double per_packet = ctx->wv.traces_per_packet > 0.0 ? 1.05 * ctx->wv.traces_per_packet : ctx->wv.log_budget_per_packet;
        s.one_set = (double)n * per_packet > 3.0 * two_set_capacity;
// ... 5 lines not shown
        log_capacity = 4000000000LL;
    }
    LogMemory m{false, 0.0, 0.0};
    bool asked = false;
    if (!ctx->wv.log_capacity_user) {
        m = log_memory(ctx);
        asked = true;
        if (m.known) log_capacity = std::min<long long>(log_capacity, (long long)(LOG_MEMORY_SHARE * m.avail / log_bytes_per_record(s.one_set ? 1 : 2, partition)));
    }
    unsigned long long cap = std::min<unsigned long long>((unsigned long long)log_capacity,
                                                          (unsigned long long)((double)n * ctx->wv.log_budget_per_packet) + 64ull * (unsigned long long)waves + 65536ull);
    if (w.n_bins > mc::EST_MAX_BINS) cap = 0;
    cap = std::min<unsigned long long>(cap, 0xfffffff0ull);
    s.region_capacity = 0;
    s.n_chunks = 0;
    if (cap > 0) {
        const unsigned long long per_wave = shell_log ? (unsigned long long)(ctx->n_shells + 4) : 4ull;
        s.region_capacity = ctx->wv.log_chunk_records > 0 ? (unsigned)ctx->wv.log_chunk_records : (shell_log ? 2048u : 4096u);
        while (s.region_capacity > 256 && (unsigned long long)s.region_capacity * per_wave * (unsigned long long)waves > cap) s.region_capacity >>= 1;
        s.region_capacity &= ~1u;
        s.n_chunks = std::max<unsigned long long>(cap / s.region_capacity, (unsigned long long)waves * ((shell_log && !ctx->wv.log_capacity_user) ? per_wave : 1ull));
        if (s.n_chunks * s.region_capacity > 0xfffffff0ull) s.n_chunks = 0xfffffff0ull / s.region_capacity;
    }
    if (s.region_capacity > 0) {
        if (!asked) m = log_memory(ctx);
        const double least = (double)waves * 256.0 * log_bytes_per_record(1, partition);
        if (m.known && least > m.avail)
            return fail(ctx, TARDIS_MC_ERR_HIP, "device memory: the tables leave %.3f GiB of %.1f GiB free, the smallest line-visit log of this call needs "
                                                "%.3f GiB", m.avail / 1073741824.0, m.total / 1073741824.0, least / 1073741824.0);
    }
    const unsigned region_capacity = s.region_capacity;
    const unsigned long long n_chunks = s.n_chunks;
    s.want_split = ctx->wv.drain_split && !vq && !s.one_set && region_capacity > 0 && n >= 64LL * waves * 4;
    s.tail_records = (double)ctx->wv.log_tail_packets * ctx->wv.traces_per_packet * 64.0 * (double)waves;
    const bool one_epoch = (double)region_capacity * (double)n_chunks >= (double)n * ctx->wv.traces_per_packet * 1.05;
    s.tail_plan = ctx->wv.log_tail_split && !vq && !s.one_set && region_capacity > 0 && ctx->wv.traces_per_packet > 0.0 && one_epoch &&
                  (double)n * ctx->wv.traces_per_packet >= 5e8 && (double)n * ctx->wv.traces_per_packet > 2.0 * s.tail_records;
    s.tail_possible = ctx->wv.log_tail_split && !vq && !s.one_set && region_capacity > 0 && (double)n * std::max(ctx->wv.traces_per_packet, 16.0) >= 5e8;
    s.want_compact = ctx->wv.drain_compact > 0 && !vq && !vpk && !cu_split && !shell_log && !s.one_set && region_capacity > 0 && n > 64LL * (waves - 1) && waves >= 8;
    const bool several_epochs = region_capacity > 0 && (unsigned long long)region_capacity * n_chunks < (unsigned long long)((double)n * ctx->wv.log_budget_per_packet);
    s.n_sets = (s.one_set || vq) ? 1 : ((s.tail_plan || s.tail_possible || s.want_split || s.want_compact || several_epochs) ? 2 : 1);
    s.set_records = (size_t)std::max<unsigned long long>((unsigned long long)region_capacity * n_chunks, 1);
    s.set1_inside = s.n_sets == 2 && !ctx->wv.log_records[1].p && ctx->wv.log_records[0].cap >= 2 * s.set_records * sizeof(mc::LineVisitRecord) &&
                    ctx->wv.log_keys[0].cap >= 2 * s.set_records * sizeof(unsigned) && (partition || ctx->wv.log_sorted[0].cap >= 2 * s.set_records * sizeof(unsigned));
    return TARDIS_MC_OK;
}

struct WaveCall {
    const PropagateCall *call;
    const WaveChoice *w;
    const LogSizing *log;
    mc::GroupArgs P;
    mc::WaveHot hot;
    int trk_defer = 0;
    long long n;
    int waves;
    bool vq, may_suspend, cu_masked, streaming;
    hipStream_t st;
    int waves_cur;
    mc::LaneSave *cur_save; mc::WaveSave *cur_wsave; uint32_t *cur_states;
    bool split_armed, compact_armed;
    bool vq_on;
    bool call_complete;
    int log_gen;
    double records_done;
    long long rs_pending_lo, rs_pending_hi;
    unsigned long long pool_chunks;
    double split_w2;
};

template <typename T> T *log_set_ptr(const LogSizing &s, const DevBuf (&buf)[2], int b) { return s.set1_inside ? buf[0].as<T>() + (size_t)b * s.set_records : buf[b].as<T>(); }

template <bool FULL, bool BINNED, typename... Args>
void launch_accumulate_as(int est_accumulate, int cus, hipStream_t es, Args... args)
{
    if (est_accumulate == 3)
        hipLaunchKernelGGL((mc::accumulate_dyadic_kernel<FULL, BINNED, true>), dim3(cus * 2), dim3(64 * mc::ACCD_WAVES), 0, es, args...);
    else if (est_accumulate == 2)
        hipLaunchKernelGGL((mc::accumulate_dyadic_kernel<FULL, BINNED>), dim3(cus), dim3(64 * mc::ACCD_WAVES), 0, es, args...);
    else if (BINNED || est_accumulate == 1)
        hipLaunchKernelGGL((mc::accumulate_blocks_kernel<FULL, BINNED>), dim3(cus * 2), dim3(64 * mc::ACCB_WAVES), 0, es, args...);
    else if constexpr (!BINNED)
        hipLaunchKernelGGL(mc::accumulate_kernel<FULL>, dim3(cus * 3), dim3(64 * mc::ACC_WAVES), 0, es, args...);
}
hipError_t launch_accumulate(bool full, bool binned, int est_accumulate, int cus, hipStream_t es, const mc::LineVisitRecord *records, const unsigned *index, const unsigned *bin_start,
                             const unsigned *slice_start, int n_bins, int tiles_per_shell, int n_lines, const double *nu_line, double *jblue_t, double *edot_t)
{
    if (full) {
        if (binned) launch_accumulate_as<true, true>(est_accumulate, cus, es, records, index, bin_start, slice_start, n_bins, tiles_per_shell, n_lines, nu_line, jblue_t, edot_t);
        else launch_accumulate_as<true, false>(est_accumulate, cus, es, records, index, bin_start, slice_start, n_bins, tiles_per_shell, n_lines, nu_line, jblue_t, edot_t);
    } else {
        if (binned) launch_accumulate_as<false, true>(est_accumulate, cus, es, records, index, bin_start, slice_start, n_bins, tiles_per_shell, n_lines, nu_line, jblue_t, edot_t);
        else launch_accumulate_as<false, false>(est_accumulate, cus, es, records, index, bin_start, slice_start, n_bins, tiles_per_shell, n_lines, nu_line, jblue_t, edot_t);
    }
    return hipGetLastError();
}

hipError_t estimator_passes(TardisMcContext *ctx, const WaveCall &E, const mc::EstimatorLog &lg, int b, hipStream_t es)
{
    if (lg.region_capacity == 0) return hipSuccess;
    const int cus = E.call->cus, n_bins = E.w->n_bins;
    const bool full = E.call->full, shell_log = E.w->key.shell_log;
    unsigned *bin_count = ctx->wv.log_bins[b].as<unsigned>(), *bin_start = bin_count + (n_bins + 1),
             *bin_fill = bin_start + (n_bins + 1), *slice_start = bin_fill + (n_bins + 1);
    hipError_t e = hipMemsetAsync(bin_count, 0, (size_t)(n_bins + 1) * sizeof(unsigned), es);
    if (e != hipSuccess) return e;
// ... 28 lines not shown
        hipLaunchKernelGGL(mc::partition_kernel<2>, dim3(part_blocks), dim3(mc::PART_THREADS), 0, es, lg.records, lg.keys, lg.region_count, lg.n_regions,
                           lg.region_capacity, (const unsigned *)nullptr, lg.tiles_per_shell, ctx->n_lines, bits_of(mc::PART_LOCAL_BUCKETS), bin_fill, scratch);
        binned = scratch;
    } else {
        hipLaunchKernelGGL(mc::partition_shell_fill_kernel, dim3(1), dim3(256), 0, es, bin_start, lg.tiles_per_shell, ctx->n_shells, shell_fill);
        hipLaunchKernelGGL(mc::partition_kernel<1>, dim3(part_blocks), dim3(mc::PART_THREADS), 0, es, lg.records, lg.keys, lg.region_count,
                           lg.n_regions, lg.region_capacity, (const unsigned *)nullptr, lg.tiles_per_shell, ctx->n_lines, bits_of(ctx->n_shells),
                           shell_fill, scratch);
        hipLaunchKernelGGL(mc::partition_kernel<0>, dim3(part_blocks), dim3(mc::PART_THREADS), 0, es, scratch, (const unsigned *)nullptr,
                           (const unsigned *)nullptr, 0, 0u, bin_start + n_bins, lg.tiles_per_shell, ctx->n_lines, bits_of(mc::PART_LOCAL_BUCKETS),
                           bin_fill, lg.records);
    }
    return launch_accumulate(full, true, ctx->wv.est_accumulate, cus, es, binned, nullptr, bin_start, slice_start, n_bins, lg.tiles_per_shell, ctx->n_lines, E.P.nu_line, E.P.jblue_t,
                             E.P.edot_t);
}

hipError_t rs_copy_pending(TardisMcContext *ctx, WaveCall &E)
{
    if (E.rs_pending_hi <= E.rs_pending_lo) return hipSuccess;
    hipError_t e = hipStreamWaitEvent(ctx->rs.stream, ctx->rs.ev, 0);
    void *dev[16];
    per_packet_device_arrays(ctx, dev);
    const size_t off = (size_t)E.rs_pending_lo * 8, bytes = (size_t)(E.rs_pending_hi - E.rs_pending_lo) * 8;
    for (int a = 0; a < 16 && e == hipSuccess; ++a)
        if (ctx->rs.dst[a] && dev[a]) e = hipMemcpyAsync((char *)ctx->rs.dst[a] + off, (char *)dev[a] + off, bytes, hipMemcpyDeviceToHost, ctx->rs.stream);
    if (e == hipSuccess) e = hipStreamSynchronize(ctx->rs.stream);
    ctx->rs.upto = E.rs_pending_hi;
    E.rs_pending_lo = E.rs_pending_hi = 0;
    return e;
}

int fill_wave_cold(TardisMcContext *ctx, const WaveCall &E, int epoch, const mc::EstimatorLog &lg, mc::WaveCold *wc_dev)
{
    const bool vq = E.vq, vpk = E.call->vpk;
    mc::WaveCold &wc = ctx->wv.wave_cold_host[epoch & 1];
    wc.P = E.P; wc.D = ctx->problem_host; wc.log = lg; wc.seeded_states = E.cur_states;
    wc.chunk_first = 0; wc.chunk_count = E.n;
    wc.launch = ctx->wv.seed_chk.as<mc::LaunchRec>();
    wc.vp_scratch = ctx->wv.vp_scratch.as<mc::VpResult>();
    wc.vp_park = (vpk && !E.vq_on && ctx->wv.vp_carry_min_active > 0) ? ctx->wv.vp_park.as<mc::VpPark>() : nullptr;
    wc.vp_carry_min_active = ctx->wv.vp_carry_min_active; wc.trk_defer = E.trk_defer;
    wc.save = E.may_suspend ? E.cur_save : nullptr;
    wc.wsave = E.may_suspend ? E.cur_wsave : nullptr;
    wc.resume = epoch > 0 ? 1 : 0;
    wc.drain_split = E.split_armed ? 64 : (E.compact_armed ? ctx->wv.drain_compact : 0);
    wc.suspended = ctx->wv.suspended_dev.as<unsigned>();
    wc.vq_req = E.vq_on ? ctx->wv.vq_req.as<mc::VolleyRequest>() : nullptr;
    wc.vq_items = E.vq_on ? ctx->wv.vq_items.as<unsigned>() : nullptr;
    wc.vq_count = vq ? ctx->wv.vq_count.as<unsigned>() : nullptr;
    wc.vq_jsave = vq ? ctx->wv.vq_jsave.as<double>() : nullptr;
    wc.log_continue = vq ? 1 : 0;
    wc.log_gen = E.log_gen;
    wc.rng_complete = ctx->wv.rng_complete;
    HIP_TRY(ctx, store_value(E.st, wc_dev, wc));
    return TARDIS_MC_OK;
}

int launch_second_half(TardisMcContext *ctx, WaveCall &E, int epoch, int waves1, hipStream_t es, mc::WaveCold *wc_dev)
{
    const mc::WaveCold &wc = ctx->wv.wave_cold_host[epoch & 1];
    mc::WaveCold wc2 = wc;
    wc2.seeded_states = wc.seeded_states + (size_t)waves1 * 64 * mc::WV_STATE_STRIDE;
    if (wc.save) wc2.save = wc.save + (size_t)waves1 * 64;
    if (wc.wsave) wc2.wsave = wc.wsave + waves1;
    if (wc.vp_scratch) wc2.vp_scratch = wc.vp_scratch + (size_t)waves1 * 64 * mc::VP_ROUND;
    if (wc.vp_park) wc2.vp_park = wc.vp_park + (size_t)waves1 * 64;
    HIP_TRY(ctx, hipStreamWaitEvent(es, ctx->wv.ev_split[0], 0));
    HIP_TRY(ctx, store_value(es, wc_dev + 1, wc2));
    HIP_TRY(ctx, hipEventRecord(ctx->wv.ev_split[1], es));
    hipLaunchKernelGGL(E.w->fn, dim3(E.waves - waves1), dim3(64), E.w->lds, es, E.hot, (const mc::WaveCold *)(wc_dev + 1));
    HIP_TRY(ctx, hipGetLastError());
    HIP_TRY(ctx, hipEventRecord(ctx->wv.ev_split[2], es));
    HIP_TRY(ctx, hipStreamWaitEvent(E.st, ctx->wv.ev_split[2], 0));
    E.split_w2 = (double)(E.waves - waves1) / (double)E.waves;
    return TARDIS_MC_OK;
}

int wave_epoch_tail_volley_queue(TardisMcContext *ctx, WaveCall &E, const mc::EstimatorLog &lg)
{
    HIP_TRY(ctx, hipEventSynchronize(ctx->ev_chunk[4]));
    float ms = 0.f;
    HIP_TRY(ctx, hipEventElapsedTime(&ms, ctx->ev_chunk[2], ctx->ev_chunk[3]));
    ctx->sum_prop_ms += ms;
    const bool last = ctx->wv.suspended_host[0] == 0;
    if (last || ctx->wv.suspended_host[1] > 0) {
        HIP_TRY(ctx, hipEventRecord(ctx->wv.ev_post[0], E.st));
        HIP_TRY(ctx, estimator_passes(ctx, E, lg, 0, E.st));
        HIP_TRY(ctx, hipEventRecord(ctx->wv.ev_post[1], E.st));
        HIP_TRY(ctx, hipMemsetAsync(lg.region_count, 0, (size_t)(E.log->n_chunks + 1) * sizeof(unsigned), E.st));
        ++E.log_gen;
        HIP_TRY(ctx, hipEventSynchronize(ctx->wv.ev_post[1]));
        HIP_TRY(ctx, hipEventElapsedTime(&ms, ctx->wv.ev_post[0], ctx->wv.ev_post[1]));
        ctx->sum_post_ms += ms;
    }
    if (last) { E.call_complete = true; return TARDIS_MC_OK; }
    const long long vq_min_items = ctx->wv.vq_min_items >= 0 ? ctx->wv.vq_min_items : (long long)E.call->cus * 4 * 64 * 8;
    if (E.vq_on && (long long)ctx->wv.suspended_host[4] < vq_min_items) E.vq_on = false;
    return TARDIS_MC_OK;
}

int wave_epoch_tail_cu_partition(TardisMcContext *ctx, WaveCall &E, const mc::EstimatorLog &lg, int b)
{
    HIP_TRY(ctx, hipEventSynchronize(ctx->ev_chunk[4]));
    float pms = 0.f;
    HIP_TRY(ctx, hipEventElapsedTime(&pms, ctx->ev_chunk[2], ctx->ev_chunk[3]));
    ctx->sum_prop_ms += pms;
// ... 257 lines not shown
    HIP_TRY(ctx, ctx->wv.suspended_dev.ensure(4 * sizeof(unsigned)));
    E.cur_save = ctx->wv.lane_save.as<mc::LaneSave>(); E.cur_wsave = ctx->wv.wave_save.as<mc::WaveSave>(); E.cur_states = ctx->wv.seeded_states.as<uint32_t>();
    if (s.want_compact) HIP_TRY(ctx, ctx->wv.drain_census.ensure(8 * sizeof(unsigned)));
    if (!ctx->wv.suspended_host) HIP_TRY(ctx, hipHostMalloc((void **)&ctx->wv.suspended_host, 16 * sizeof(unsigned), hipHostMallocDefault));
    if (vq) {
        HIP_TRY(ctx, ctx->wv.vq_req.ensure((size_t)waves * 64 * sizeof(mc::VolleyRequest)));
        HIP_TRY(ctx, ctx->wv.vq_items.ensure((size_t)waves * 64 * mc::VP_ROUND * sizeof(unsigned)));
        HIP_TRY(ctx, ctx->wv.vq_count.ensure(2 * sizeof(unsigned)));
        HIP_TRY(ctx, ctx->wv.vq_jsave.ensure((size_t)waves * 2 * (size_t)ctx->n_shells * sizeof(double)));
        if ((size_t)waves * 64 >= (1u << 29)) return fail(ctx, TARDIS_MC_ERR_INVALID_ARGUMENT, "too many lanes for the volley queue's item words");
    }
    if (vpk) HIP_TRY(ctx, ctx->wv.vp_scratch.ensure((size_t)waves * 64 * mc::VP_ROUND * sizeof(mc::VpResult)));
    if (vpk && ctx->wv.vp_carry_min_active > 0) HIP_TRY(ctx, ctx->wv.vp_park.ensure((size_t)waves * 64 * sizeof(mc::VpPark)));
    HIP_TRY(ctx, ctx->wv.wave_cold_dev.ensure(4 * sizeof(mc::WaveCold)));
    ctx->wv.wave_cold_host.resize(2);
    for (hipEvent_t &e : ctx->wv.ev_split)
        if (!e) HIP_TRY(ctx, hipEventCreate(&e));
    hipStream_t st = ctx->stream;
    HIP_TRY(ctx, hipEventRecord(ctx->ev_start, st));
    if (call.tune_slot >= 0) HIP_TRY(ctx, hipEventRecord(ctx->lt.ev_tune[0], st));
    if (E.cu_masked) {
        HIP_TRY(ctx, hipEventRecord(ctx->wv.ev_fork_m, ctx->stream));
        st = ctx->wv.stream_prop_m;
        HIP_TRY(ctx, hipStreamWaitEvent(st, ctx->wv.ev_fork_m, 0));
    }
    E.st = st;
    HIP_TRY(ctx, hipEventRecord(ctx->ev_chunk[0], st));
    if (n > 0) {
        mc::LaunchPrepArgs la{};
        la.r0 = F.r0; la.mu0 = F.mu0; la.nu0 = F.nu0; la.e0 = F.e0; la.nu_line = P.nu_line;
        la.seeds = ctx->pk.seeds.as<uint32_t>();
        la.bucket_first = P.bucket_first; la.bucket_shift = P.bucket_shift; la.bucket_n = P.bucket_n; la.n_lines = P.n_lines;
        la.bucket_kmin = P.bucket_kmin; la.t_exp = P.t_exp;
        la.out = ctx->wv.seed_chk.as<mc::LaunchRec>(); la.first = 0; la.count = n;
        if (full) hipLaunchKernelGGL(mc::launch_prep_kernel<true>, dim3((unsigned)((n + 255) / 256)), dim3(256), 0, st, la);
        else hipLaunchKernelGGL(mc::launch_prep_kernel<false>, dim3((unsigned)((n + 255) / 256)), dim3(256), 0, st, la);
        HIP_TRY(ctx, hipGetLastError());
    }
    HIP_TRY(ctx, hipEventRecord(ctx->ev_chunk[1], st));
    E.P = P;
    mc::WaveHot &hot = E.hot;
    hot.nu_line = P.nu_line; hot.tau_t = w.key.nt ? P.nt_t : P.tau_t; hot.n_lines = P.n_lines; hot.n_shells = P.n_shells;
    hot.disable_line_scattering = P.disable_line_scattering; hot.debug_flags = P.debug_flags;
    hot.t_exp = P.t_exp;
    const bool mostly_hot = ctx->wt.have_hot && 2 * ctx->wt.n_hot_blocks > (long long)ctx->n_levels;
    hot.ls_min_active = (!ctx->wv.ls_min_active_user && mostly_hot) ? 12 : ctx->wv.ls_min_active;
    hot.ls_max_steps = ctx->wv.ls_max_steps;
    hot.walk_min_active = (!ctx->wv.walk_min_active_user && mostly_hot) ? 16 : ctx->wv.walk_min_active;
    hot.vq_min_active = ctx->wv.vq_min_active;
    {
        const WaveKernelKey &k = w.key;
        const bool has_defer = k.track && k.lane_sweep && !k.vpk && !k.full_tracking && !k.xwalk;
        const bool fits = mc::tracker_pack_fits(P.n_shells, P.n_lines) && (ctx->wv.tracker_pack_max_lines <= 0 || P.n_lines <= ctx->wv.tracker_pack_max_lines);
        E.trk_defer = (has_defer && ctx->wv.tracker_defer && fits) ? 1 : 0;
        ctx->wv.last_tracker_defer = has_defer ? E.trk_defer : -1;
    }
    hot.line_block = P.line_interaction_type != 0 ? P.line_block : nullptr;
    ctx->wv.post_pending[0] = ctx->wv.post_pending[1] = false;
    ctx->wv.prop_pending = false;
    E.streaming = call.rs_armed && !vq && !E.cu_masked && E.may_suspend && n >= ctx->rs.min_packets;
    if (E.streaming) {
        ctx->rs.late_capacity = (unsigned)std::min<long long>(n, (long long)waves * 64 * 16);
        HIP_TRY(ctx, ctx->rs.late.ensure((size_t)ctx->rs.late_capacity * sizeof(unsigned)));
        HIP_TRY(ctx, ctx->rs.late_count.ensure(sizeof(unsigned)));
        HIP_TRY(ctx, hipMemsetAsync(ctx->rs.late_count.p, 0, sizeof(unsigned), st));
        if (!ctx->rs.stream) HIP_TRY(ctx, hipStreamCreateWithFlags(&ctx->rs.stream, hipStreamNonBlocking));
        if (!ctx->rs.ev) HIP_TRY(ctx, hipEventCreateWithFlags(&ctx->rs.ev, hipEventDisableTiming));
        if (!ctx->rs.next_host) HIP_TRY(ctx, hipHostMalloc((void **)&ctx->rs.next_host, sizeof(unsigned long long), hipHostMallocDefault));
    }
    const int max_epochs = 1 << 20;
    E.vq_on = vq;
    E.call_complete = n <= 0;
    for (int epoch = 0; n > 0 && epoch < max_epochs && !E.call_complete; ++epoch)
        if ((rc = run_wave_epoch(ctx, E, epoch))) return rc;
    if (E.streaming && E.call_complete) HIP_TRY(ctx, rs_copy_pending(ctx, E));
    if (!E.call_complete)
        return fail(ctx, TARDIS_MC_ERR_STATE, "propagate: %d launches did not finish the call (waves still suspended)", max_epochs);
    if (E.cu_masked) {
        HIP_TRY(ctx, hipEventRecord(ctx->wv.ev_join, ctx->wv.stream_pass_m));
        HIP_TRY(ctx, hipStreamWaitEvent(ctx->stream, ctx->wv.ev_join, 0));
        HIP_TRY(ctx, hipEventRecord(ctx->wv.ev_join_m, st));
        HIP_TRY(ctx, hipStreamWaitEvent(ctx->stream, ctx->wv.ev_join_m, 0));
    } else if (s.n_sets == 2 && (ctx->wv.post_pending[0] || ctx->wv.post_pending[1])) {
        HIP_TRY(ctx, hipEventRecord(ctx->wv.ev_join, ctx->wv.stream2));
        HIP_TRY(ctx, hipStreamWaitEvent(ctx->stream, ctx->wv.ev_join, 0));
    }
    ctx->wv.wave_epoch_mode = true;
    ctx->pg.progress_done = true;
    long long unpack_from = 0;
    if (E.streaming && ctx->rs.upto > 0 && (rc = gather_late_results(ctx, &unpack_from))) return rc;
    if (ctx->pk.track && n > unpack_from) {
        hipLaunchKernelGGL(mc::tracker_unpack_kernel, dim3((unsigned)((n - unpack_from + 255) / 256)), dim3(256), 0, ctx->stream, F, unpack_from, n - unpack_from,
                           (const unsigned *)nullptr);
        HIP_TRY(ctx, hipGetLastError());
    }
    return TARDIS_MC_OK;
}

int run_group_kernel(TardisMcContext *ctx, const PropagateCall &call, const mc::GroupArgs &P)
{
    const bool vpk = call.vpk;
    const int cus = call.cus;
    ctx->wv.wave_epoch_mode = false;
    long long chunk = std::min<long long>(std::max<long long>(ctx->pk.n_packets, 1), ctx->chunk_packets);
    HIP_TRY(ctx, ctx->wv.seeded_states.ensure((size_t)chunk * mc::WV_STATE_STRIDE * sizeof(uint32_t)));
    const int G = ctx->group_size == 8 ? 8 : (ctx->group_size == 16 ? 16 : ((ctx->n_lines <= 100000 && !vpk) ? 8 : 16));
// ... 154 lines not shown
    if (!ctx || !name) return TARDIS_MC_ERR_INVALID_ARGUMENT;
    std::string n(name);
    if (n == "variant") ctx->variant = (int)value;
    else if (n == "blocks_per_cu") ctx->blocks_per_cu = std::max(1, (int)value);
    else if (n == "track_last_interaction") ctx->pk.track = value != 0;
    else if (n == "estimator_copies") { ctx->es.est_copies = std::max(1, std::min(8, (int)value)); ctx->es.est_valid = false; }
    else if (n == "vpacket_log_capacity") { ctx->vl.vlog_capacity = value; ctx->vl.vlog_capacity_user = value > 0; }
    else if (n == "track_full") ctx->el.track_full = value != 0;
    else if (n == "vpacket_last_interaction") ctx->vl.vlog_li = value != 0;
    else if (n == "event_log_capacity") ctx->el.evlog_capacity = std::max<long long>(0, value);
    else if (n == "event_log_max_bytes") ctx->el.evlog_max_bytes = std::max<long long>(1LL << 20, value);
    else if (n == "debug_flags") ctx->debug_flags = (int)value;
    else if (n == "drain_split") ctx->wv.drain_split = value ? 1 : 0;
    else if (n == "drain_compact") ctx->wv.drain_compact = (int)std::max<long long>(0, std::min<long long>(48, value));
    else if (n == "est_one_level") ctx->wv.est_one_level = value ? 1 : 0;
    else if (n == "drain_pack_lanes") ctx->wv.drain_pack_lanes = (int)std::max<long long>(1, std::min<long long>(64, value));
    else if (n == "walk_sector_packing") ctx->wt.walk_sector_packing = value ? 1 : 0;
    else if (n == "walk_hot") ctx->wt.walk_hot = value < 0 ? -1 : (value ? 1 : 0);
    else if (n == "walk_hot_min_mass") ctx->wt.walk_hot_min_mass = (int)std::max<long long>(0, std::min<long long>(value, 1001));
    else if (n == "walk_hot_min_mass_long") ctx->wt.walk_hot_min_mass_long = (int)std::max<long long>(0, std::min<long long>(value, 1001));
    else if (n == "vpacket_screening") ctx->sc.vpacket_screening = value < 0 ? -1 : (value ? 1 : 0);
    else if (n == "waves_per_simd") ctx->waves_per_simd = (int)value;
    else if (n == "lane_sweep_min_active") {
        ctx->wv.ls_min_active_user = value >= 0;
        ctx->wv.ls_min_active = value >= 0 ? (int)std::min<long long>(value, 63) : 8;
    }
    else if (n == "lane_sweep_max_steps") ctx->wv.ls_max_steps = (int)std::max<long long>(1, value);
    else if (n == "vq_oversubscribe") ctx->wv.vq_oversubscribe = (int)std::max<long long>(1, std::min<long long>(value, 64));
    else if (n == "vq_tracer_waves_per_simd") ctx->wv.vq_tracer_waves_per_simd = (int)std::max<long long>(1, std::min<long long>(value, 16));
    else if (n == "vq_min_items") ctx->wv.vq_min_items = value;
    else if (n == "vq_min_active") ctx->wv.vq_min_active = (int)std::max<long long>(0, std::min<long long>(value, 63));
    else if (n == "log_tail_split") ctx->wv.log_tail_split = value ? 1 : 0;
    else if (n == "est_pipeline") ctx->wv.est_pipeline = value ? 1 : 0;
    else if (n == "pass_cus") ctx->wv.pass_cus = (int)std::max<long long>(0, std::min<long long>(value, 16));
    else if (n == "vpk_wave_min_packets") ctx->vpk_wave_min_packets = std::max<long long>(0, value);
    else if (n == "ls_waves_per_simd") { ctx->lt.ls_waves_per_simd = (value == 3 || value == 4) ? (int)value : 0; ctx->lt.ls_tune.n = -1; }
    else if (n == "epoch_split") ctx->wv.epoch_split = value ? 1 : 0;
    else if (n == "log_by_shell") ctx->wv.log_by_shell = value < 0 ? -1 : (value ? 1 : 0);
    else if (n == "stream_min_packets") ctx->rs.min_packets = std::max<long long>(64, value);
    else if (n == "sweep_table") ctx->sw.sweep_table = (int)std::max<long long>(-1, std::min<long long>(value, 2));
    else if (n == "table_offsets") ctx->table_offsets = value < 0 ? -1 : (value ? 1 : 0);
    else if (n == "vpk_wide_registers") ctx->vpk_wide_registers = (int)std::max<long long>(0, std::min<long long>(value, 2));
    else if (n == "bucket_lines_permille") ctx->ot.bucket_lines_permille = (int)std::max<long long>(50, std::min<long long>(value, 16000));
    else if (n == "vp_carry_min_active") ctx->wv.vp_carry_min_active = (int)std::max<long long>(0, std::min<long long>(value, 63));
    else if (n == "est_accumulate") ctx->wv.est_accumulate = (int)std::max<long long>(0, std::min<long long>(value, 3));
    else if (n == "log_tail_packets") ctx->wv.log_tail_packets = (int)std::max<long long>(0, std::min<long long>(value, 1000));
    else if (n == "log_chunk_records") ctx->wv.log_chunk_records = value <= 0 ? 0 : std::max<long long>(256, std::min<long long>(value, 1 << 20));
    else if (n == "walk_min_active") {
        ctx->wv.walk_min_active_user = value >= -1;
        ctx->wv.walk_min_active = value >= -1 ? (int)std::min<long long>(value, 63) : 8;
    }
    else if (n == "tracker_defer") ctx->wv.tracker_defer = value ? 1 : 0;
    else if (n == "rng_complete") ctx->wv.rng_complete = value ? 1 : 0;
    else if (n == "tracker_pack_max_lines") ctx->wv.tracker_pack_max_lines = std::max<long long>(0, value);
    else if (n == "group_size") ctx->group_size = (value == 4 || value == 8 || value == 16) ? (int)value : 0;
    else if (n == "pipeline_chunks") {}
    else if (n == "log_capacity") { ctx->wv.log_capacity = std::max<long long>(0, value); ctx->wv.log_capacity_user = true; }
    else if (n == "log_sets") ctx->wv.log_sets = (value == 1 || value == 2) ? (int)value : 0;
    else if (n == "source_max_iterations") ctx->sf.max_iterations = std::max<long long>(1, value);
    else if (n == "chunk_packets") ctx->chunk_packets = std::max<long long>(1024, value);
    else if (n == "opacity_update_long_rows") ctx->ou.long_rows = value < 0 ? -1 : value;
    else if (n == "plasma_update_long_rows") ctx->pl.long_rows = value < 0 ? -1 : value;
    else if (n == "plasma_max_iterations") ctx->pl.max_iterations = std::max<long long>(1, value);
    else if (n == "nlte_lds_levels") ctx->nl.lds_levels = value < 0 ? -1 : value;
    else if (n == "nlte_blocked_levels") ctx->nl.blocked_levels = value < 0 ? -1 : value;
    else return fail(ctx, TARDIS_MC_ERR_INVALID_ARGUMENT, "unknown option '%s'", name);
    return TARDIS_MC_OK;
}

int tardis_mc_set_geometry(TardisMcContext *ctx, const TardisMcGeometry *g)
{
    if (!ctx || !g || g->n_shells <= 0 || !g->r_inner || !g->r_outer)
        return fail(ctx, TARDIS_MC_ERR_INVALID_ARGUMENT, "invalid geometry");
    HIP_TRY(ctx, hipSetDevice(ctx->device));
    drop_products(ctx, GEOMETRY_REPLACED);
    int rc;
    if ((rc = upload(ctx, ctx->r_inner, g->r_inner, (size_t)g->n_shells))) return rc;
    if ((rc = upload(ctx, ctx->r_outer, g->r_outer, (size_t)g->n_shells))) return rc;
    HIP_TRY(ctx, hipStreamSynchronize(ctx->stream));
    ctx->n_shells = (int)g->n_shells;
    ctx->t_exp = g->time_explosion;
    ctx->have_geometry = true;
    return TARDIS_MC_OK;
}

static int derive_opacity_tables(TardisMcContext *ctx, const size_t L, const size_t S, const size_t T, const std::function<void(const char *)> &tmark)
{
    const std::vector<int> &l2l = ctx->ot.h_idx[0], &edge = ctx->ot.h_idx[1], &ttype = ctx->ot.h_idx[2], &dest = ctx->ot.h_idx[3], &tline = ctx->ot.h_idx[4];
    const std::vector<double> &nu = ctx->ot.h_nu;
    const bool macro = ctx->ot.h_macro;
    const size_t E = macro ? edge.size() : 1;
    int rc;
    drop_products(ctx, OPACITY_VALUES_REPLACED);
    {
        HIP_TRY(ctx, ctx->ot.cum_t.ensure((T * S + 8) * sizeof(double)));
        HIP_TRY(ctx, hipMemcpyAsync(ctx->ot.cum_t.p, ctx->ot.prob_t.p, T * S * sizeof(double), hipMemcpyDeviceToDevice, ctx->stream));
        ctx->ot.prob_negative = false;
        if (macro && E > 1) {
            HIP_TRY(ctx, ctx->sc.pfx_flag.ensure(sizeof(int)));
            int *flag = ctx->sc.pfx_flag.as<int>();
            HIP_TRY(ctx, hipMemsetAsync(flag, 0, sizeof(int), ctx->stream));
            const long long n = (long long)(E - 1) * (long long)S;
            hipLaunchKernelGGL(mc::macro_cumulative_kernel, dim3((unsigned)((n + 255) / 256)), dim3(256), 0, ctx->stream, ctx->ot.prob_t.as<double>(),
                               ctx->ot.cum_t.as<double>(), ctx->ot.block_edge.as<int>(), (int)(E - 1), (long long)T, (int)S, flag);
            int neg = 0;
            hipError_t e1 = hipGetLastError();
// ... 512 lines not shown
    PropagateCall call{};
    call.vpk = c.number_of_vpackets > 0;
    call.full = c.enable_full_relativity != 0;
    call.cus = ctx->prop.multiProcessorCount > 0 ? ctx->prop.multiProcessorCount : 256;
    call.rs_armed = ctx->rs.armed;
    ctx->rs.armed = false; ctx->rs.upto = 0; ctx->rs.n_late = 0;
    call.tune_pending = ctx->lt.ls_tune.pending;
    ctx->lt.ls_tune.pending = -1;
    call.tune_slot = -1;
    int rc = ensure_estimators(ctx);
    if (rc) return rc;
    if (!ctx->counters.p) {
        HIP_TRY(ctx, ctx->counters.ensure(TARDIS_MC_N_COUNTERS * sizeof(unsigned long long)));
        HIP_TRY(ctx, hipMemsetAsync(ctx->counters.p, 0, TARDIS_MC_N_COUNTERS * sizeof(unsigned long long), ctx->stream));
    }
    if (ctx->pk.track) {
        const size_t P = (size_t)std::max<long long>(ctx->pk.n_packets, 1);
        for (auto &b : ctx->pk.li_f64) HIP_TRY(ctx, b.ensure(P * sizeof(double)));
        for (auto &b : ctx->pk.li_i64) HIP_TRY(ctx, b.ensure(P * sizeof(long long)));
        HIP_TRY(ctx, ctx->pk.li_rec.ensure(P * 64));
    }
    if (ctx->el.track_full) HIP_TRY(ctx, ctx->pk.li_rec.ensure((size_t)std::max<long long>(ctx->pk.n_packets, 1) * 64));
    if (c.enable_vpacket_tracking && call.vpk) {
        if (!ctx->vl.vlog_capacity_user) ctx->vl.vlog_capacity = std::max<long long>(1024, ctx->pk.n_packets * c.number_of_vpackets * 64);
        size_t cap = (size_t)ctx->vl.vlog_capacity;
        HIP_TRY(ctx, ctx->vl.vlog_count.ensure(sizeof(unsigned long long)));
        HIP_TRY(ctx, hipMemsetAsync(ctx->vl.vlog_count.p, 0, sizeof(unsigned long long), ctx->stream));
        HIP_TRY(ctx, ctx->vl.vlog_packet.ensure(cap * sizeof(long long)));
        HIP_TRY(ctx, ctx->vl.vlog_seq.ensure(cap * sizeof(int)));
        HIP_TRY(ctx, ctx->vl.vlog_nu.ensure(cap * sizeof(double)));
        HIP_TRY(ctx, ctx->vl.vlog_energy.ensure(cap * sizeof(double)));
        HIP_TRY(ctx, ctx->vl.vlog_mu.ensure(cap * sizeof(double)));
        HIP_TRY(ctx, ctx->vl.vlog_r.ensure(cap * sizeof(double) * (vlog_li_call(ctx) ? 4 : 1)));
    }
    HIP_TRY(ctx, ctx->first_error.ensure(2 * sizeof(long long)));
    HIP_TRY(ctx, store_value(ctx->stream, ctx->first_error.as<FirstErrorInit>(), FirstErrorInit{{0x7fffffffffffffffLL, 0}}));
    ctx->pg.progress_done = false; ctx->pg.progress_wave = false; ctx->pg.progress_total = ctx->pk.n_packets;
    {
        std::lock_guard<std::mutex> lock(ctx->pg.progress_mutex);
        HIP_TRY(ctx, ctx->next_packet.ensure(sizeof(unsigned long long)));
        if (!ctx->pg.ev_progress_reset) HIP_TRY(ctx, hipEventCreateWithFlags(&ctx->pg.ev_progress_reset, hipEventDisableTiming));
    }
    HIP_TRY(ctx, hipMemsetAsync(ctx->next_packet.p, 0, sizeof(unsigned long long), ctx->stream));
    HIP_TRY(ctx, hipEventRecord(ctx->pg.ev_progress_reset, ctx->stream));
    call.plan = plan::plan_propagate(plan_input(ctx));
    if (!call.plan.error && call.plan.screen_on && !ctx->sc.pfx_valid) {
        rc = build_screening_tables(ctx);
        if (rc) return rc;
        if (ctx->sc.pfx_negative) call.plan = plan::plan_propagate(plan_input(ctx));
    }
    if (call.plan.error) return fail(ctx, call.plan.error, "%s", call.plan.message);
    ctx->last_table_offsets = call.plan.last_table_offsets;
    ctx->last_variant = call.plan.last_variant;
    ctx->wv.last_tracker_defer = -1;
    ctx->last_kernel_table = -1;
    std::fill(std::begin(ctx->last_kernel_key), std::end(ctx->last_kernel_key), 0);
    rc = call.plan.cooperative ? run_cooperative(ctx, call) : run_lane_kernel(ctx, call);
    if (rc) return rc;
    {
        if (!ctx->wv.events_host) {
            HIP_TRY(ctx, hipHostMalloc((void **)&ctx->wv.events_host, 2 * sizeof(unsigned long long), hipHostMallocDefault));
            ctx->wv.events_host[0] = ctx->wv.events_host[1] = 0;
            HIP_TRY(ctx, hipEventCreateWithFlags(&ctx->wv.ev_events, hipEventDisableTiming));
        }
        ctx->wv.events_host[1] = (unsigned long long)ctx->pk.n_packets;
        HIP_TRY(ctx, hipMemcpyAsync(&ctx->wv.events_host[0], ctx->counters.as<unsigned long long>() + TARDIS_MC_CNT_EVENTS,
                                    sizeof(unsigned long long), hipMemcpyDeviceToHost, ctx->stream));
        HIP_TRY(ctx, hipEventRecord(ctx->wv.ev_events, ctx->stream));
    }
    HIP_TRY(ctx, hipEventRecord(ctx->ev_stop, ctx->stream));
    ctx->timed = true;
    ctx->es.est_propagated = true;
    if (call.tune_slot >= 0) {
        HIP_TRY(ctx, hipEventRecord(ctx->lt.ev_tune[1], ctx->stream));
        ctx->lt.ls_tune.pending = call.tune_slot;
    }
    ctx->el.ev_valid = ctx->el.track_full;
    ctx->pk.li_valid = ctx->pk.track;
    ctx->vl.vl_valid = c.enable_vpacket_tracking && call.vpk && ctx->vl.vlog_capacity > 0;
    ctx->vl.vl_li = vlog_li_call(ctx);
    ctx->vl.vl_packets = ctx->pk.n_packets;
    ctx->vl.vl_capacity = ctx->vl.vlog_capacity;
    return TARDIS_MC_OK;
}

int tardis_mc_synchronize(TardisMcContext *ctx)
{
    if (!ctx) return TARDIS_MC_ERR_INVALID_ARGUMENT;
    HIP_TRY(ctx, hipSetDevice(ctx->device));
    HIP_TRY(ctx, hipStreamSynchronize(ctx->stream));
    ctx->pg.progress_done = true;
    return TARDIS_MC_OK;
}

int tardis_mc_progress(TardisMcContext *ctx, int64_t *out_packets_started, int64_t *out_packets_total)
{
    if (!ctx || !out_packets_started || !out_packets_total) return TARDIS_MC_ERR_INVALID_ARGUMENT;
    const long long total = ctx->pg.progress_total.load();
    *out_packets_total = total;
    *out_packets_started = 0;
    if (ctx->pg.progress_done.load()) { *out_packets_started = total; return TARDIS_MC_OK; }
    if (!ctx->pg.progress_wave.load()) return TARDIS_MC_OK;
    std::lock_guard<std::mutex> lock(ctx->pg.progress_mutex);
    if (hipSetDevice(ctx->device) != hipSuccess) return TARDIS_MC_ERR_HIP;
    if (!ctx->next_packet.p || !ctx->pg.ev_progress_reset || hipEventQuery(ctx->pg.ev_progress_reset) != hipSuccess) return TARDIS_MC_OK;
    if (!ctx->pg.stream_progress && hipStreamCreateWithFlags(&ctx->pg.stream_progress, hipStreamNonBlocking) != hipSuccess) return TARDIS_MC_ERR_HIP;
// ... 32 lines not shown
            HIP_TRY(ctx, hipEventElapsedTime(&ms, ctx->ev_chunk[2], ctx->ev_chunk[3]));
            ctx->sum_prop_ms += ms;
            ctx->wv.prop_pending = false;
        }
        for (int b = 0; b < 2; ++b)
            if (ctx->wv.post_pending[b]) {
                HIP_TRY(ctx, hipEventSynchronize(ctx->wv.ev_post[2 * b + 1]));
                HIP_TRY(ctx, hipEventElapsedTime(&ms, ctx->wv.ev_post[2 * b], ctx->wv.ev_post[2 * b + 1]));
                ctx->sum_post_ms += ms;
                ctx->wv.post_pending[b] = false;
            }
        ctx->last_post_ms = ctx->sum_post_ms;
        if (out_seed_ms) *out_seed_ms = ctx->sum_seed_ms;
        if (out_propagate_ms) *out_propagate_ms = ctx->sum_prop_ms;
        if (out_launches) *out_launches = std::max(ctx->launches, 1);
        return TARDIS_MC_OK;
    }
    if (ctx->chunks_timed == 0) {
        float ms = 0.f;
        HIP_TRY(ctx, hipEventElapsedTime(&ms, ctx->ev_start, ctx->ev_stop));
        prop = ms;
    }
    double post = 0.0;
    for (int ci = 0; ci < ctx->chunks_timed; ++ci) {
        float a = 0.f, b = 0.f, c = 0.f;
        HIP_TRY(ctx, hipEventElapsedTime(&a, ctx->ev_chunk[4 * ci], ctx->ev_chunk[4 * ci + 1]));
        HIP_TRY(ctx, hipEventElapsedTime(&b, ctx->ev_chunk[4 * ci + 1], ctx->ev_chunk[4 * ci + 2]));
        HIP_TRY(ctx, hipEventElapsedTime(&c, ctx->ev_chunk[4 * ci + 2], ctx->ev_chunk[4 * ci + 3]));
        seed += a;
        prop += b;
        post += c;
    }
    ctx->last_post_ms = post;
    if (out_seed_ms) *out_seed_ms = seed;
    if (out_propagate_ms) *out_propagate_ms = prop;
    if (out_launches) *out_launches = ctx->chunks_timed ? ctx->chunks_timed : 1;
    return TARDIS_MC_OK;
}

int tardis_mc_last_counters(TardisMcContext *ctx, int64_t out_counters[TARDIS_MC_N_COUNTERS])
{
    if (!ctx || !out_counters) return TARDIS_MC_ERR_INVALID_ARGUMENT;
    if (!ctx->counters.p) return fail(ctx, TARDIS_MC_ERR_STATE, "no work counters yet");
    HIP_TRY(ctx, hipSetDevice(ctx->device));
    unsigned long long cnt[TARDIS_MC_N_COUNTERS];
    HIP_TRY(ctx, hipMemcpyAsync(cnt, ctx->counters.p, sizeof cnt, hipMemcpyDeviceToHost, ctx->stream));
    HIP_TRY(ctx, hipStreamSynchronize(ctx->stream));
    for (int k = 0; k < TARDIS_MC_N_COUNTERS; ++k) out_counters[k] = (int64_t)cnt[k];
    out_counters[TARDIS_MC_CNT_PACKETS] = ctx->pk.n_packets;
    return TARDIS_MC_OK;
}

int tardis_mc_last_variant(TardisMcContext *ctx) { return ctx ? ctx->last_variant : -1; }
int tardis_mc_last_table_offsets(TardisMcContext *ctx) { return ctx ? ctx->last_table_offsets : -1; }
int tardis_mc_last_compactions(TardisMcContext *ctx) { return ctx ? ctx->wv.compactions : -1; }
int tardis_mc_last_tracker_defer(TardisMcContext *ctx) { return ctx ? ctx->wv.last_tracker_defer : -1; }

int tardis_mc_kernel_table_row(int table, int row, int key[12])
{
    if (table == 0) return kernel_table_row(LANE_KERNELS, row, key);
    if (table == 1) return kernel_table_row(GROUP_KERNELS, row, key);
    if (table == 2) return kernel_table_row(WAVE_KERNELS, row, key);
    return TARDIS_MC_ERR_INVALID_ARGUMENT;
}

int tardis_mc_last_kernel_key(TardisMcContext *ctx, int *table, int key[12])
{
    if (!ctx || !table || !key) return TARDIS_MC_ERR_INVALID_ARGUMENT;
    *table = ctx->last_kernel_table;
    std::copy(std::begin(ctx->last_kernel_key), std::end(ctx->last_kernel_key), key);
    return TARDIS_MC_OK;
}

int tardis_mc_last_estimator_ms(TardisMcContext *ctx, double *out_ms)
{
    if (!ctx || !out_ms) return TARDIS_MC_ERR_INVALID_ARGUMENT;
    double seed, prop;
    int launches;
    int rc = tardis_mc_last_kernel_times(ctx, &seed, &prop, &launches);
    if (rc) return rc;
    *out_ms = ctx->last_post_ms;
    return TARDIS_MC_OK;
}

static int reduce_estimator_copies(TardisMcContext *ctx)
{
    if (ctx->es.est_copies <= 1) return TARDIS_MC_OK;
    EstLayout e = est_layout(ctx->es.est_S, ctx->es.est_L, ctx->es.est_G, ctx->es.est_copies);
    long long n = (long long)(2 * ctx->es.est_S * ctx->es.est_L);
    hipLaunchKernelGGL(reduce_copies_kernel, dim3(2048), dim3(256), 0, ctx->stream, ctx->es.est.as<double>() + e.jblue, n,
                       (long long)e.copy_stride, ctx->es.est_copies);
    HIP_TRY(ctx, hipGetLastError());
    return TARDIS_MC_OK;
}

int tardis_mc_get_results(TardisMcContext *ctx, TardisMcResult *res)
{
    if (!ctx || !res) return TARDIS_MC_ERR_INVALID_ARGUMENT;
    if (!ctx->es.est_valid) return fail(ctx, TARDIS_MC_ERR_STATE, "nothing to fetch");
    HIP_TRY(ctx, hipSetDevice(ctx->device));
    int rc = reduce_estimator_copies(ctx);
    if (rc) return rc;
    const size_t P = (size_t)ctx->pk.n_packets, S = ctx->es.est_S, L = ctx->es.est_L, G = ctx->es.est_G;
    EstLayout e = est_layout(S, L, G, ctx->es.est_copies);
    double *base = ctx->es.est.as<double>();
    auto d2h = [&](void *dst, const void *src, size_t bytes) -> hipError_t {
// ... 1952 lines not shown
```

tardis_amd/csrc/tau_prefix.hpp:

```cpp
#pragma once
#include <hip/hip_runtime.h>

namespace mc {

struct DD { double hi, lo; };
__device__ __forceinline__ void dd_add(DD &a, double x)
{
    const double s = a.hi + x;
    const double bb = s - a.hi;
    const double err = (a.hi - (s - bb)) + (x - bb);
    a.hi = s;
    a.lo += err;
}
__device__ __forceinline__ void dd_add_dd(DD &a, const DD &b)
{
    dd_add(a, b.hi);
    a.lo += b.lo;
}

__global__ void __launch_bounds__(256) tau_prefix_kernel(const double *__restrict__ tau_t, int n_lines, double *__restrict__ pfx,
                                                         double *__restrict__ rowsum, int *__restrict__ negative)
{
    __shared__ DD part[256];
    const int s = blockIdx.x, tid = threadIdx.x;
    const double *__restrict__ row = tau_t + (size_t)s * (size_t)n_lines;
    double *__restrict__ out = pfx + (size_t)s * (size_t)(n_lines + 1);
    const int per = (n_lines + 255) / 256;
    const int i0 = min(tid * per, n_lines), i1 = min(i0 + per, n_lines);
    DD acc = {0.0, 0.0};
    bool neg = false;
    for (int i = i0; i < i1; ++i) {
        const double x = row[i];
        neg |= !(x >= 0.0);
        dd_add(acc, x);
    }
    part[tid] = acc;
    __syncthreads();
    if (tid == 0) {
        DD run = {0.0, 0.0};
        for (int k = 0; k < 256; ++k) {
            const DD t = part[k];
            part[k] = run;
            dd_add_dd(run, t);
        }
        rowsum[s] = run.hi + run.lo;
    }
    __syncthreads();
    acc = part[tid];
    for (int i = i0; i < i1; ++i) {
        out[i] = acc.hi + acc.lo;
        dd_add(acc, row[i]);
    }
    if (i1 == n_lines && i0 < n_lines) out[n_lines] = acc.hi + acc.lo;
    if (n_lines == 0 && tid == 0) out[0] = 0.0;
    if (neg) atomicOr(negative, 1);
}

}
```

tardis_amd/engine.py:

```python
from __future__ import annotations

import ctypes as C

import numpy as np

from . import _abi, _lib
from . import state as st


class MonteCarloException(ValueError):
    """Mirror of tardis.transport.montecarlo.utils.MonteCarloException (utils.py:9)."""


class MacroAtomError(ValueError):
    """Mirror of tardis.transport.montecarlo.macro_atom.MacroAtomError (macro_atom.py:15)."""


class EventLogOverflow(RuntimeError):

    def __init__(self, rows_needed: int, dropped: int):
        super().__init__(f"full r-packet log overflow: {dropped} of {rows_needed} rows dropped; re-run with "
                         f"event_log_capacity={rows_needed}")
        self.rows_needed, self.dropped = int(rows_needed), int(dropped)

# ... 288 lines not shown

    def progress(self) -> tuple[int, int]:
        a, b = C.c_int64(), C.c_int64()
        self._check(self._L.tardis_mc_progress(self._h, C.byref(a), C.byref(b)), "progress")
        return int(a.value), int(b.value)

    def last_propagate_ms(self) -> float:
        v = C.c_double()
        self._check(self._L.tardis_mc_last_propagate_ms(self._h, C.byref(v)), "last_propagate_ms")
        return v.value

    def last_kernel_times(self) -> dict:
        a, b, n = C.c_double(), C.c_double(), C.c_int()
        self._check(self._L.tardis_mc_last_kernel_times(self._h, C.byref(a), C.byref(b), C.byref(n)), "last_kernel_times")
        e = C.c_double()
        self._check(self._L.tardis_mc_last_estimator_ms(self._h, C.byref(e)), "last_estimator_ms")
        return {"seed_ms": a.value, "propagate_ms": b.value, "launches": n.value, "estimator_ms": e.value}

    def last_compactions(self) -> int:
        return int(self._L.tardis_mc_last_compactions(self._h))

    def last_tracker_defer(self) -> int:
        return int(self._L.tardis_mc_last_tracker_defer(self._h))

    KERNEL_TABLES = ("lane", "group", "wave")
    KERNEL_KEY_FIELDS = {"lane": ("FULL", "VPK", "TRACK", "FT", "VLI"),
                         "group": ("FULL", "TRACK", "G", "BLOCK", "OCC", "VPK", "WIDE", "VLI"),
                         "wave": ("FULL", "TRACK", "G", "VPK", "LS", "XWALK", "WPE", "NT", "SL", "FT", "WIDE", "VLI")}

    @staticmethod
    def kernel_table(table: str) -> list:
        L, t = _lib.lib(), Engine.KERNEL_TABLES.index(table)
        key = (C.c_int * 12)()
        n = L.tardis_mc_kernel_table_row(t, -1, key)
        if n < 0:
            raise RuntimeError(f"tardis_mc_kernel_table_row({table}) failed ({n})")
        width = len(Engine.KERNEL_KEY_FIELDS[table])
        rows = []
        for r in range(n):
            L.tardis_mc_kernel_table_row(t, r, key)
            rows.append(tuple(key[:width]))
        return rows

    def last_kernel_key(self):
        t, key = C.c_int(-1), (C.c_int * 12)()
        self._check(self._L.tardis_mc_last_kernel_key(self._h, C.byref(t), key), "last_kernel_key")
        if t.value < 0:
            return None, ()
        table = self.KERNEL_TABLES[t.value]
        return table, tuple(key[:len(self.KERNEL_KEY_FIELDS[table])])

    def last_variant(self) -> int:
        return int(self._L.tardis_mc_last_variant(self._h))

    def last_table_offsets(self) -> int:
        return int(self._L.tardis_mc_last_table_offsets(self._h))

    def get_event_log(self) -> st.FullTrackers:
        probe = _abi.TardisMcEventLog()
        offsets = np.zeros(self.n_packets + 1, dtype=np.int64)
        probe.offsets = _abi._ip(offsets)
        self._check(self._L.tardis_mc_get_event_log(self._h, C.byref(probe)), "get_event_log")
        if probe.dropped:
            raise EventLogOverflow(probe.count, probe.dropped)
        n = int(probe.count)
        cols = {f: np.empty(n) for f in _abi._EV_F64}
        cols.update({f: np.empty(n, dtype=np.int64) for f in _abi._EV_I64})
        log = _abi.TardisMcEventLog()
        log.capacity = n
        for f in _abi._EV_F64:
            setattr(log, f, _abi._dp(cols[f]))
        for f in _abi._EV_I64:
            setattr(log, f, _abi._ip(cols[f]))
        self._check(self._L.tardis_mc_get_event_log(self._h, C.byref(log)), "get_event_log")
        return st.FullTrackers(offsets, cols)

    def get_vpacket_log(self) -> st.VPacketCollection:
        probe = _abi.TardisMcVpacketLog()
        self._check(self._L.tardis_mc_get_vpacket_log(self._h, C.byref(probe)), "get_vpacket_log")
        n = int(probe.count)
        vt = st.VPacketCollection(-1, None, None, None, self._n_v, n)
        vt.offsets = np.zeros(self.n_packets + 1, dtype=np.int64)
        vt.source_packet = np.empty(n, dtype=np.int64)
        log = _abi.TardisMcVpacketLog()
        log.capacity = n
        log.offsets, log.source_packet = _abi._ip(vt.offsets), _abi._ip(vt.source_packet)
        f64, i64 = _abi._VL_F64, _abi._VL_I64
        if not self.options.get("vpacket_last_interaction", 0):
            f64, i64 = f64[:4], ()
        for f in f64:
            setattr(log, f, _abi._dp(getattr(vt, f)))
        for f in i64:
            setattr(log, f, _abi._ip(getattr(vt, f)))
        vt.offsets[-1] = -1
        self._check(self._L.tardis_mc_get_vpacket_log(self._h, C.byref(log)), "get_vpacket_log")
        if vt.offsets[-1] != n:
            raise VPacketLogOverflow(n)
        return vt

    def get_results(self, output_nus=None, output_energies=None, track_last_interaction=True,
                    want_line_estimators=True, vpacket_log_capacity=None, want_packet_outputs=True, trackers=None,
                    track_full=False) -> _abi.ResultBuffers:
        if not track_last_interaction:
            trackers = None
        elif not (isinstance(trackers, st.LastInteractionTrackers) and len(trackers) == self.n_packets):
            trackers = st.LastInteractionTrackers(self.n_packets)
# ... 277 lines not shown
```

Baseline: 37.70 million packets/s.

## Add coarse block-skip line sweep using prefix-sum tau tables

Builds a coarse table of per-8-line blocks (last nu and prefix-summed tau) plus a per-shell prefix table, and lets the lane sweep jump over whole blocks when a conservative bound shows no interaction inside them. A follow-up interval mode confirms the found event against a rounding margin and otherwise falls back to the exact fine sweep from the starting line. This is meant to cut the per-line memory loads and compares of long line walks across 500k lines. In exchange it adds table-building kernels and a host sync, extra state on suspension, and a fallback path whose correctness depends on the margin bound.

```diff
diff --git a/include/tardis_mc.h b/include/tardis_mc.h
--- a/include/tardis_mc.h
+++ b/include/tardis_mc.h
@@ -159,6 +159,7 @@
 int tardis_mc_last_estimator_ms(TardisMcContext *ctx, double *out_ms);
 int tardis_mc_last_counters(TardisMcContext *ctx, int64_t out_counters[TARDIS_MC_N_COUNTERS]);
 int tardis_mc_last_variant(TardisMcContext *ctx);
+int tardis_mc_last_sweep_skip(TardisMcContext *ctx);
 int tardis_mc_last_table_offsets(TardisMcContext *ctx);
 int tardis_mc_last_compactions(TardisMcContext *ctx);
 int tardis_mc_last_tracker_defer(TardisMcContext *ctx);
diff --git a/tardis_amd/_lib.py b/tardis_amd/_lib.py
--- a/tardis_amd/_lib.py
+++ b/tardis_amd/_lib.py
@@ -30,6 +30,7 @@
     "tardis_mc_last_estimator_ms": (_i, [_vp, C.POINTER(C.c_double)]),
     "tardis_mc_last_counters": (_i, [_vp, C.POINTER(C.c_int64)]),
     "tardis_mc_last_variant": (_i, [_vp]),
+    "tardis_mc_last_sweep_skip": (_i, [_vp]),
     "tardis_mc_last_table_offsets": (_i, [_vp]),
     "tardis_mc_last_compactions": (_i, [_vp]),
     "tardis_mc_last_tracker_defer": (_i, [_vp]),
diff --git a/tardis_amd/csrc/propagate_plan.hpp b/tardis_amd/csrc/propagate_plan.hpp
--- a/tardis_amd/csrc/propagate_plan.hpp
+++ b/tardis_amd/csrc/propagate_plan.hpp
@@ -8,6 +8,7 @@
 constexpr int DBG_WALK_GROUP_FP64 = 8192;
 constexpr int DBG_LONG_INSTANTIATIONS = 1048576;
 constexpr int DBG_NO_SCREENING = 33554432;
+constexpr int DBG_SKIP_FALLBACK = 536870912;
 constexpr int DBG_WAVE_COUNTERS = 1 | 2 | 4 | 16 | 32 | 16384 | 32768 | 65536 | 131072 | 524288 | 2097152 | 4194304 | 8388608 | 16777216 | 134217728 | 268435456;
 constexpr int DBG_FP64_WALKS = DBG_WALK_LANE_FP64 | DBG_WALK_GROUP_FP64;
 constexpr int DBG_WAVE_CROSS_CHECK = DBG_FP64_WALKS | DBG_LONG_INSTANTIATIONS | DBG_WAVE_COUNTERS;
@@ -101,4 +102,18 @@
     return p;
 }
 
+struct SkipInput {
+    int sweep_skip;
+    bool lane_sweep, vpk, full_relativity, wide, cross_check, shell_log, full_tracking;
+    int waves_per_simd, nt;
+    bool line_scattering;
+    bool nt_negative, pfx_negative;
+};
+inline bool plan_sweep_skip(const SkipInput &in)
+{
+    if (in.sweep_skip == 0) return false;
+    return in.lane_sweep && !in.vpk && !in.full_relativity && !in.wide && !in.cross_check && !in.shell_log && !in.full_tracking && in.waves_per_simd == 4 &&
+           in.nt == 1 && in.line_scattering && !in.nt_negative && !in.pfx_negative;
 }
+
+}
diff --git a/tardis_amd/csrc/propagate_wave.hpp b/tardis_amd/csrc/propagate_wave.hpp
--- a/tardis_amd/csrc/propagate_wave.hpp
+++ b/tardis_amd/csrc/propagate_wave.hpp
@@ -5,6 +5,7 @@
 #include "walk_tables.hpp"
 #include "event_log.hpp"
 #include "mt_generation.hpp"
+#include "sweep_skip.hpp"
 
 namespace mc {
 
@@ -116,6 +117,9 @@
     int log_gen;
     double *vq_jsave;
     int rng_complete;
+    int sweep_skip;
+    unsigned sk_ct_off, sk_pn_off;
+    double sk_margin;
 };
 
 __global__ void __launch_bounds__(64) late_list_kernel(const LaneSave *__restrict__ save, const WaveSave *__restrict__ wsave, int waves, long long first, long long end,
@@ -312,6 +316,9 @@
 #define TMC_LS_CHUNK_NT 10
 #endif
 constexpr int LS_CHUNK_NT = TMC_LS_CHUNK_NT;
+#ifndef TMC_SWEEP_SKIP
+#define TMC_SWEEP_SKIP 1
+#endif
 
 __global__ void __launch_bounds__(256) macro_cumulative_kernel(const double *__restrict__ prob_t, double *__restrict__ cum_t,
                                                                 const int *__restrict__ block_edge, int n_blocks, long long n_trans,
@@ -652,6 +659,7 @@
     static_assert(NT != 2 || WPE != 3, "aligned runs are eight lines long");
     constexpr bool DEFER = TRACK && LS && !VPK && !FT && !XWALK;
     constexpr bool RNGC = LS && !VPK;
+    constexpr bool SKIP = TMC_SWEEP_SKIP != 0 && LS && !VPK && NT == 1 && WPE == 4 && !WIDE && !SL && !XWALK && !FULL && !FT && TMC_STRAIGHT_A == 0;
     extern __shared__ __attribute__((aligned(16))) unsigned char lds_raw[];
     WaveShared &sh = *reinterpret_cast<WaveShared *>(lds_raw);
     constexpr size_t SH_BYTES = LS ? WAVE_SHARED_LS_BYTES : sizeof(WaveShared);
@@ -910,6 +918,11 @@
             v.vseq = vseq; v.pred_bits = pred_bits; v.vdone = vq_done; v.pad_v0 = v.pad_v1 = v.pad_v2 = 0;
             v.walk_inv_new = sh.chi[lane]; v.walk_block = sh.rcp_chi[lane]; v.walk_event = sh.tau_event[lane]; v.pad_w = 0.0;
             v.trk_nu = sh.nu[lane]; v.trk_mu = sh.rcp_nu[lane]; v.trk_energy = sh.comov_nu[lane];
+            if constexpr (SKIP) {
+                if (s_active && (pflags & (ssk::MODE_COARSE | ssk::MODE_INTERVAL))) {
+                    v.s_line = p.next_line_id; v.s_tau = 0.0; v.pflags = (pflags & ~ssk::MODE_INTERVAL) | ssk::MODE_COARSE;
+                }
+            }
             suspended = true;
             break;
         }
@@ -1730,6 +1743,9 @@
                     s_xb = ((d_boundary * p.nu) * P.rcp_tc) * (1.0 - 0x1p-40);
                     s_fast = fast && mid_range(s_kp);
                     s_active = true;
+                    if constexpr (SKIP) {
+                        if (W->sweep_skip && s_fast) pflags |= ssk::MODE_COARSE;
+                    }
                 } else {
                     sh.nu[lane] = p.nu; sh.rcp_nu[lane] = 1.0 / p.nu; sh.comov_nu[lane] = comov_nu;
                     sh.chi[lane] = chi_e; sh.rcp_chi[lane] = 1.0 / chi_e;
@@ -1768,7 +1784,18 @@
                     const unsigned nt_at = s_row + (unsigned)s_line;
                     const nt2 *__restrict__ pq = reinterpret_cast<const nt2 *>(H.tau_t) + (NT == 2 ? (nt_at & ~7u) : nt_at);
                     const int k0 = NT == 2 ? (int)(nt_at & 7u) : 0;
-                    if constexpr (NT != 0) {
+                    if constexpr (SKIP) {
+                        unsigned at = nt_at, last = nt_at + (unsigned)(CH - 1);
+                        if (pflags & ssk::MODE_COARSE) {
+                            last = W->sk_pn_off + (unsigned)p.shell * (unsigned)(L + 1) + (unsigned)p.next_line_id;
+                            at = W->sk_ct_off + (nt_at >> 3);
+                        }
+                        const nt2 *__restrict__ pc = reinterpret_cast<const nt2 *>(H.tau_t) + at;
+#pragma unroll
+                        for (int k = 0; k < CH - 1; ++k) { const nt2 e = pc[k]; nl[k] = e.x; tl[k] = e.y; }
+                        const nt2 e = reinterpret_cast<const nt2 *>(H.tau_t)[last];
+                        nl[CH - 1] = e.x; tl[CH - 1] = e.y;
+                    } else if constexpr (NT != 0) {
 #pragma unroll
                         for (int k = 0; k < CH; ++k) { const nt2 e = pq[k]; nl[k] = e.x; tl[k] = e.y; }
                     } else {
@@ -1784,6 +1811,19 @@
                     const int n_fast = L - 1 - s_line;
                     bool alive;
                     double f_nu, f_tau;
+                    if (SKIP && (pflags & ssk::MODE_COARSE)) {
+                        if constexpr (SKIP) {
+                            double hi;
+                            const int c = ssk::coarse_scan(nl, tl, comov, s_kp, s_xb, s_tau_event, W->sk_margin, hi);
+                            const int b = s_line >> 3;
+                            if (c == ssk::STEP) s_line = (b + ssk::ADVANCE) << 3;
+                            else if (c > 0) { s_line = (b + c) << 3; s_tau = hi; pflags ^= ssk::MODE_COARSE | ssk::MODE_INTERVAL; }
+                            else {
+                                s_line = p.next_line_id; s_tau = 0.0; pflags &= ~ssk::MODE_COARSE;
+                            }
+                        }
+                        alive = true; f_nu = 0.0; f_tau = 0.0;
+                    } else
                     if constexpr ((WPE == 3 && !VPK) || (TMC_STRAIGHT_A != 0 && WPE == 4 && NT == 1)) {
                         double t[CH + 1];
                         t[0] = s_tau;
@@ -1850,12 +1890,21 @@
                         double dist;
                         if (line < L) {
                             code = lane_exact_line(H, line, f_nu, f_tau, s_tau, p.nu, comov, chi, s_tau_event, d_bound, dist);
+                            if constexpr (SKIP) {
+                                if ((pflags & ssk::MODE_INTERVAL) && code &&
+                                    !ssk::interval_take(code, s_tau, W->sweep_skip == 2 ? __builtin_inf() : ssk::GAP_FACTOR * W->sk_margin, f_tau, chi, dist, s_tau_event)) {
+                                    code = 0; f_tau = 0.0; s_tau = 0.0; adv = p.next_line_id - s_line - 1; pflags &= ~ssk::MODE_INTERVAL;
+                                }
+                            }
                             if (!code) { s_tau = s_tau + f_tau; ++adv; }
                         } else {
                             const double d_cont = (s_tau_event - s_tau) / chi;
                             const bool cont = d_cont < d_bound;
                             dist = cont ? d_cont : d_bound;
                             code = (cont ? 2 : 1) | 8;
+                            if constexpr (SKIP) {
+                                if ((pflags & ssk::MODE_INTERVAL) && cont) { code = 0; s_tau = 0.0; adv = p.next_line_id - s_line; pflags &= ~ssk::MODE_INTERVAL; }
+                            }
                         }
                         if (code) {
                             sh.d_boundary[lane] = dist; sh.res_info[lane] = code; sh.res_line[lane] = (code & 8) ? 0 : line;
diff --git a/tardis_amd/csrc/sweep_skip.hpp b/tardis_amd/csrc/sweep_skip.hpp
--- /dev/null
+++ b/tardis_amd/csrc/sweep_skip.hpp
@@ -0,0 +1,153 @@
+#pragma once
+
+#if defined(__HIPCC__)
+#define SSK_FN __host__ __device__ inline
+#else
+#define SSK_FN inline
+#endif
+
+namespace ssk {
+
+constexpr int BLOCK = 8;
+constexpr int LOADS = 10;
+constexpr int STEP = 9;
+constexpr int ADVANCE = 8;
+constexpr double GAP_FACTOR = 8.0;
+constexpr int MODE_COARSE = 8, MODE_INTERVAL = 16;
+
+struct Entry { double nu_last, p_end; };
+
+SSK_FN double margin(int n_lines, double rowsum_max)
+{
+    return rowsum_max * (1.02 * ((double)n_lines + 16.0) * 0x1p-53 + 0x1p-48);
+}
+
+SSK_FN int coarse_scan(const double (&nu_last)[LOADS], const double (&p_end)[LOADS], double comov, double kp, double xb, double tau_event, double m, double &hi)
+{
+    int c = 0;
+    const double p_start = p_end[STEP];
+    const double x_start = comov - nu_last[STEP];
+    bool alive = x_start >= 0.0 && x_start < xb;
+    double h_keep = 0.0;
+#if defined(__HIPCC__)
+#pragma unroll
+#endif
+    for (int k = 0; k < STEP; ++k) {
+        const double d = p_end[k] - p_start;
+        const double h = d + m;
+        const double X = comov - nu_last[k];
+        const double x = kp * X;
+        const double sum = h + x;
+        alive = alive && X < xb && sum < tau_event;
+        if (alive) { c = k + 1; h_keep = h; }
+    }
+    hi = h_keep;
+    return c;
+}
+
+SSK_FN bool interval_take(int code, double u, double g, double tau_line, double chi, double dist, double tau_event)
+{
+    if (!(g < __builtin_inf())) return false;
+    if (code == 1) return true;
+    if (code != 3) return false;
+    const double lo = u - g;
+    const double incl = lo + tau_line;
+    const double cd = chi * dist;
+    return incl + cd > tau_event;
+}
+
+#if !defined(__HIPCC__)
+struct TraceIn {
+    const double *nt, *ct, *pn;
+    int n_lines, start;
+    double nu, comov, chi, tau_event, d_boundary, kp, xb, t_exp, m;
+    int force_fallback, skip, fine_chunk;
+};
+struct TraceOut { int code, line; double dist; int fell_back, coarse_steps, fine_steps, interval, fb_code; double fb_gap; int fb_line; double fb_u; };
+
+constexpr double C_LIGHT_ = 2.99792458e10, MISS_ = 1e99, CLOSE_ = 1e-14;
+inline int exact_line(int L, double t_exp, int line, double nu_line, double tau_line, double tau_prev, double nu, double comov_nu, double chi, double tau_event,
+                      double d_boundary, double &distance)
+{
+    const double tau_incl = tau_prev + tau_line;
+    const double d_cont = (tau_event - tau_prev) / chi;
+    const bool is_last = line == L - 1;
+    const double nu_diff = comov_nu - nu_line;
+    const double q = nu_diff / nu;
+    const bool close = (q < 0 ? -q : q) < CLOSE_;
+    const bool err = !is_last && !close && !(nu_diff >= 0);
+    const double d_far = q * C_LIGHT_ * t_exp;
+    const double d_trace = is_last ? MISS_ : (close ? 0.0 : d_far);
+    const double tau_combined = tau_incl + chi * d_trace;
+    double dmin = d_trace;
+    if (d_boundary < dmin) dmin = d_boundary;
+    if (d_cont < dmin) dmin = d_cont;
+    const bool stop_b = !err && d_trace != 0 && dmin == d_boundary;
+    const bool stop_e = !err && d_trace != 0 && !stop_b && dmin == d_cont;
+    const bool stop_l = !err && !stop_b && !stop_e && tau_combined > tau_event;
+    distance = stop_b ? d_boundary : (stop_e ? d_cont : d_trace);
+    return stop_b ? 1 : (stop_e ? 2 : (stop_l ? 3 : (err ? 4 : 0)));
+}
+
+inline TraceOut trace(const TraceIn &in, const double *nu_true)
+{
+    TraceOut out{};
+    const int L = in.n_lines, CH = in.fine_chunk;
+    int mode = in.skip ? MODE_COARSE : 0;
+    int s_line = in.start;
+    double s_tau = 0.0;
+    const double g = in.force_fallback ? __builtin_inf() : GAP_FACTOR * in.m;
+    for (;;) {
+        if (mode & MODE_COARSE) {
+            ++out.coarse_steps;
+            double nl[LOADS], pe[LOADS], hi;
+            const int b = s_line >> 3;
+            for (int k = 0; k < STEP; ++k) { nl[k] = in.ct[2 * (b + k)]; pe[k] = in.ct[2 * (b + k) + 1]; }
+            nl[STEP] = in.pn[2 * in.start]; pe[STEP] = in.pn[2 * in.start + 1];
+            const int c = coarse_scan(nl, pe, in.comov, in.kp, in.xb, in.tau_event, in.m, hi);
+            const bool first = s_line == in.start;
+            if (c == STEP) s_line = (b + ADVANCE) << 3;
+            else if (c > 0) { s_line = (b + c) << 3; s_tau = hi; mode = MODE_INTERVAL; out.interval = 1; }
+            else if (first) mode = 0;
+            else { s_line = in.start; s_tau = 0.0; mode = 0; out.fell_back = 1; }
+            continue;
+        }
+        ++out.fine_steps;
+        int adv = 0;
+        bool alive = true;
+        double f_nu = in.nt[2 * s_line], f_tau = in.nt[2 * s_line + 1];
+        for (int k = 0; k < CH && alive; ++k) {
+            const double nuk = in.nt[2 * (s_line + k)], tk = in.nt[2 * (s_line + k) + 1];
+            const double X = in.comov - nuk, x = in.kp * X, tau_n = s_tau + tk, sum = tau_n + x;
+            const bool ok = (k > 0 || X >= 0.0) && X < in.xb && sum < in.tau_event;
+            if (ok) { s_tau = tau_n; adv = k + 1; }
+            else { alive = false; f_nu = nuk; f_tau = tk; }
+        }
+        if (!alive) {
+            const int line = s_line + adv;
+            int code;
+            double dist;
+            if (line < L) {
+                code = exact_line(L, in.t_exp, line, line < L - 1 ? f_nu : nu_true[line], f_tau, s_tau, in.nu, in.comov, in.chi, in.tau_event, in.d_boundary, dist);
+                if ((mode & MODE_INTERVAL) && code && !interval_take(code, s_tau, g, f_tau, in.chi, dist, in.tau_event)) {
+                    out.fb_code = code; out.fb_line = line; out.fb_u = s_tau;
+                    out.fb_gap = code == 3 ? ((s_tau + f_tau) + in.chi * dist) - in.tau_event : (s_tau + in.chi * dist) - in.tau_event;
+                    code = -1;
+                }
+                if (!code) { s_tau = s_tau + f_tau; ++adv; }
+            } else {
+                const double d_cont = (in.tau_event - s_tau) / in.chi;
+                const bool cont = d_cont < in.d_boundary;
+                dist = cont ? d_cont : in.d_boundary;
+                code = (cont ? 2 : 1) | 8;
+                if ((mode & MODE_INTERVAL) && cont) { out.fb_code = code; out.fb_line = L; out.fb_u = s_tau; out.fb_gap = (s_tau + in.chi * dist) - in.tau_event; code = -1; }
+            }
+            if (code < 0) { s_line = in.start; adv = 0; s_tau = 0.0; mode = 0; out.fell_back = 1; }
+            else if (code) { out.code = code; out.line = (code & 8) ? 0 : line; out.dist = dist; return out; }
+        }
+        s_line += adv;
+    }
+}
+#endif
+
+}
diff --git a/tardis_amd/csrc/tardis_mc_hip.hip b/tardis_amd/csrc/tardis_mc_hip.hip
--- a/tardis_amd/csrc/tardis_mc_hip.hip
+++ b/tardis_amd/csrc/tardis_mc_hip.hip
@@ -27,6 +27,7 @@
 #include "formal_interpolate.hpp"
 #include "source_function.hpp"
 #include "tau_prefix.hpp"
+#include "sweep_skip.hpp"
 #include "propagate_plan.hpp"
 #include "packet_decomposition.hpp"
 #include "decomposition_plan.hpp"
@@ -203,7 +204,12 @@
         DevBuf nt_t;
         bool nt_valid = false, nt_negative = false;
         unsigned nt_stride = 0;
-        void release() { release_buffers(nt_t); }
+        int sweep_skip = -1, last_sweep_skip = 0;
+        bool sk_valid = false, sk_negative = false;
+        unsigned sk_ct_off = 0, sk_pn_off = 0;
+        double sk_margin = 0.0;
+        DevBuf sk_rowsum;
+        void release() { release_buffers(nt_t, sk_rowsum); }
     } sw;
     struct Estimators {
         DevBuf est;
@@ -459,6 +465,24 @@
     if (neg) atomicOr(negative, 1);
 }
 
+__global__ void __launch_bounds__(256) coarse_table_kernel(const double2 *__restrict__ nt, double2 *__restrict__ pn, double2 *__restrict__ ct, long long L,
+                                                           long long S, long long stride, long long total)
+{
+    const long long rows = stride / 8;
+    for (long long i = (long long)blockIdx.x * blockDim.x + threadIdx.x; i < total; i += (long long)gridDim.x * blockDim.x) {
+        const long long s = i / rows, b = i - s * rows;
+        if (s < S) {
+            const long long e = 8 * b + 8 < L ? 8 * b + 8 : L;
+            ct[i] = make_double2(nt[s * stride + 8 * b + 7].x, pn[s * (L + 1) + e].y);
+        } else
+            ct[i] = make_double2(-__builtin_inf(), pn[(S - 1) * (L + 1) + L].y);
+    }
+    for (long long i = (long long)blockIdx.x * blockDim.x + threadIdx.x; i < S * (L + 1); i += (long long)gridDim.x * blockDim.x) {
+        const long long s = i / (L + 1), l = i - s * (L + 1);
+        pn[i].x = l < L - 1 ? nt[s * stride + l].x : -__builtin_inf();
+    }
+}
+
 template <typename T>
 __global__ void store_value_kernel(T *dst, const T v)
 {
@@ -798,6 +822,7 @@
         ctx->wt.have_walk_tables = ctx->wt.have_hot = false;
         ctx->sc.pfx_valid = false;
         ctx->sw.nt_valid = false;
+        ctx->sw.sk_valid = false;
         break;
     case CONFIG_REPLACED: ctx->vl.vl_valid = ctx->vl.vl_consolidated = false; break;
     case PACKETS_REPLACED:
@@ -1131,12 +1156,19 @@
     return TARDIS_MC_OK;
 }
 
-int build_sweep_table(TardisMcContext *ctx)
+size_t skip_table_bytes(const TardisMcContext *ctx)
+{
+    const size_t stride = ((size_t)ctx->n_lines + 7) & ~(size_t)7;
+    return ((stride / 8) * (size_t)ctx->n_shells + 16) * 16 + ((size_t)ctx->n_shells * ((size_t)ctx->n_lines + 1) + 1) * 16;
+}
+
+int build_sweep_table(TardisMcContext *ctx, bool skip_room)
 {
     const unsigned long long stride = ((unsigned long long)ctx->n_lines + 7ull) & ~7ull;
     if (ctx->sw.nt_valid || stride * (unsigned long long)ctx->n_shells + 32ull >= (1ull << 28)) return TARDIS_MC_OK;
     const long long total = (long long)(stride * (unsigned long long)ctx->n_shells) + 32;
-    HIP_TRY(ctx, ctx->sw.nt_t.ensure((size_t)total * 16));
+    HIP_TRY(ctx, ctx->sw.nt_t.ensure((size_t)total * 16 + (skip_room ? skip_table_bytes(ctx) : 0)));
+    ctx->sw.sk_valid = false;
     HIP_TRY(ctx, ctx->sc.pfx_flag.ensure(sizeof(int)));
     HIP_TRY(ctx, hipMemsetAsync(ctx->sc.pfx_flag.p, 0, sizeof(int), ctx->stream));
     hipLaunchKernelGGL(interleave_kernel, dim3((unsigned)std::min<long long>((total + 255) / 256, 65536)), dim3(256), 0, ctx->stream, ctx->ot.nu_line.as<double>(),
@@ -1149,6 +1181,45 @@
     ctx->sw.nt_negative = neg != 0;
     ctx->sw.nt_stride = (unsigned)stride;
     ctx->sw.nt_valid = true;
+    return TARDIS_MC_OK;
+}
+
+int build_skip_tables(TardisMcContext *ctx)
+{
+    if (ctx->sw.sk_valid || !ctx->sw.nt_valid) return TARDIS_MC_OK;
+    const size_t S = (size_t)ctx->n_shells, L = (size_t)ctx->n_lines, stride = ctx->sw.nt_stride;
+    const size_t nt_total = stride * S + 32, ct_rows = stride / 8, ct_total = ct_rows * S + 16;
+    if (ctx->sw.nt_t.cap < nt_total * 16 + skip_table_bytes(ctx)) {
+        ctx->sw.nt_valid = false;
+        int rc = build_sweep_table(ctx, true);
+        if (rc) return rc;
+        if (!ctx->sw.nt_valid) return TARDIS_MC_OK;
+    }
+    double2 *nt = ctx->sw.nt_t.as<double2>();
+    double2 *ct = nt + nt_total;
+    double2 *pn = ct + ct_total;
+    HIP_TRY(ctx, ctx->sw.sk_rowsum.ensure(S * sizeof(double)));
+    HIP_TRY(ctx, ctx->sc.pfx_flag.ensure(sizeof(int)));
+    HIP_TRY(ctx, hipMemsetAsync(ctx->sc.pfx_flag.p, 0, sizeof(int), ctx->stream));
+    hipLaunchKernelGGL(mc::tau_prefix_kernel, dim3((unsigned)S), dim3(256), 0, ctx->stream, ctx->ot.tau_t.as<double>(), (int)L, reinterpret_cast<double *>(pn),
+                       ctx->sw.sk_rowsum.as<double>(), ctx->sc.pfx_flag.as<int>(), 2, 1);
+    HIP_TRY(ctx, hipGetLastError());
+    hipLaunchKernelGGL(coarse_table_kernel, dim3((unsigned)std::min<size_t>((S * (L + 1) + 255) / 256, 65536)), dim3(256), 0, ctx->stream, (const double2 *)nt,
+                       pn, ct, (long long)L, (long long)S, (long long)stride, (long long)ct_total);
+    HIP_TRY(ctx, hipGetLastError());
+    int neg = 0;
+    std::vector<double> rowsum(S);
+    HIP_TRY(ctx, hipMemcpyAsync(&neg, ctx->sc.pfx_flag.p, sizeof(int), hipMemcpyDeviceToHost, ctx->stream));
+    HIP_TRY(ctx, hipMemcpyAsync(rowsum.data(), ctx->sw.sk_rowsum.p, S * sizeof(double), hipMemcpyDeviceToHost, ctx->stream));
+    HIP_TRY(ctx, hipStreamSynchronize(ctx->stream));
+    double r_max = 0.0;
+    bool finite = true;
+    for (double r : rowsum) { finite = finite && r >= 0.0 && r < 1e300; if (r > r_max) r_max = r; }
+    ctx->sw.sk_negative = neg != 0 || !finite;
+    ctx->sw.sk_margin = ssk::margin((int)L, r_max);
+    ctx->sw.sk_ct_off = (unsigned)nt_total;
+    ctx->sw.sk_pn_off = (unsigned)(nt_total + ct_total);
+    ctx->sw.sk_valid = true;
     return TARDIS_MC_OK;
 }
 
@@ -1197,6 +1268,7 @@
     int waves_per_cu;
     int max_waves_per_cu;
     bool compact_walk, ls3;
+    int sweep_skip;
     int tiles, n_bins;
     bool partition;
 };
@@ -1226,7 +1298,10 @@
         if (rc) return rc;
         if (w.ls3) k.waves_per_simd = 3;
         if (!w64 && ctx->sw.sweep_table != 0) {
-            rc = build_sweep_table(ctx);
+            plan::SkipInput room{};
+            room.sweep_skip = ctx->sw.sweep_skip; room.lane_sweep = true; room.full_relativity = full; room.full_tracking = ctx->el.track_full;
+            room.waves_per_simd = k.waves_per_simd; room.nt = (ctx->sw.sweep_table == 2 && !w.ls3) ? 2 : 1; room.line_scattering = !c.disable_line_scattering;
+            rc = build_sweep_table(ctx, plan::plan_sweep_skip(room));
             if (rc) return rc;
             if (ctx->sw.nt_valid && !ctx->sw.nt_negative) {
                 k.nt = (ctx->sw.sweep_table == 2 && !w.ls3) ? 2 : 1;
@@ -1240,6 +1315,21 @@
     w.partition = ctx->wv.est_pipeline == 1 && w.tiles <= mc::PART_LOCAL_BUCKETS && ctx->n_shells <= mc::PART_LOCAL_BUCKETS;
     k.shell_log = k.lane_sweep && !vpk && !k.xwalk && !w64 && !vq && w.partition && ctx->wv.log_by_shell != 0 && ctx->n_shells <= 64 &&
                   ((!w.ls3 && k.nt == 1) || (w.ls3 && k.nt == 0));
+    w.sweep_skip = 0;
+    if (TMC_SWEEP_SKIP != 0) {
+        plan::SkipInput si{};
+        si.sweep_skip = ctx->sw.sweep_skip; si.lane_sweep = k.lane_sweep; si.vpk = vpk; si.full_relativity = full; si.wide = w64; si.cross_check = k.xwalk;
+        si.shell_log = k.shell_log; si.full_tracking = ctx->el.track_full; si.waves_per_simd = k.waves_per_simd; si.nt = k.nt;
+        si.line_scattering = !c.disable_line_scattering; si.nt_negative = ctx->sw.nt_negative; si.pfx_negative = false;
+        if (plan::plan_sweep_skip(si)) {
+            int rc = build_skip_tables(ctx);
+            if (rc) return rc;
+            P.nt_t = ctx->sw.nt_t.as<double>(); P.nt_stride = ctx->sw.nt_stride;
+            si.pfx_negative = !ctx->sw.sk_valid || ctx->sw.sk_negative;
+            if (plan::plan_sweep_skip(si)) w.sweep_skip = (ctx->debug_flags & plan::DBG_SKIP_FALLBACK) ? 2 : 1;
+        }
+        ctx->sw.last_sweep_skip = w.sweep_skip ? 1 : 0;
+    }
     if (ctx->el.track_full) {
         k.full_tracking = true; k.track = true; k.width = 16;
     }
@@ -1351,6 +1441,7 @@
     const LogSizing *log;
     mc::GroupArgs P;
     mc::WaveHot hot;
+    int sweep_skip = 0;
     int trk_defer = 0;
     long long n;
     int waves;
@@ -1485,6 +1576,7 @@
     wc.log_continue = vq ? 1 : 0;
     wc.log_gen = E.log_gen;
     wc.rng_complete = ctx->wv.rng_complete;
+    wc.sweep_skip = E.sweep_skip; wc.sk_ct_off = ctx->sw.sk_ct_off; wc.sk_pn_off = ctx->sw.sk_pn_off; wc.sk_margin = ctx->sw.sk_margin;
     HIP_TRY(ctx, store_value(E.st, wc_dev, wc));
     return TARDIS_MC_OK;
 }
@@ -1848,6 +1940,7 @@
         const WaveKernelKey &k = w.key;
         const bool has_defer = k.track && k.lane_sweep && !k.vpk && !k.full_tracking && !k.xwalk;
         const bool fits = mc::tracker_pack_fits(P.n_shells, P.n_lines) && (ctx->wv.tracker_pack_max_lines <= 0 || P.n_lines <= ctx->wv.tracker_pack_max_lines);
+        E.sweep_skip = w.sweep_skip;
         E.trk_defer = (has_defer && ctx->wv.tracker_defer && fits) ? 1 : 0;
         ctx->wv.last_tracker_defer = has_defer ? E.trk_defer : -1;
     }
@@ -2108,6 +2201,7 @@
     }
     else if (n == "tracker_defer") ctx->wv.tracker_defer = value ? 1 : 0;
     else if (n == "rng_complete") ctx->wv.rng_complete = value ? 1 : 0;
+    else if (n == "sweep_skip") ctx->sw.sweep_skip = (int)std::max<long long>(-1, std::min<long long>(value, 1));
     else if (n == "tracker_pack_max_lines") ctx->wv.tracker_pack_max_lines = std::max<long long>(0, value);
     else if (n == "group_size") ctx->group_size = (value == 4 || value == 8 || value == 16) ? (int)value : 0;
     else if (n == "pipeline_chunks") {}
@@ -2726,6 +2820,7 @@
     if (call.plan.error) return fail(ctx, call.plan.error, "%s", call.plan.message);
     ctx->last_table_offsets = call.plan.last_table_offsets;
     ctx->last_variant = call.plan.last_variant;
+    ctx->sw.last_sweep_skip = 0;
     ctx->wv.last_tracker_defer = -1;
     ctx->last_kernel_table = -1;
     std::fill(std::begin(ctx->last_kernel_key), std::end(ctx->last_kernel_key), 0);
@@ -2864,6 +2959,7 @@
 }
 
 int tardis_mc_last_variant(TardisMcContext *ctx) { return ctx ? ctx->last_variant : -1; }
+int tardis_mc_last_sweep_skip(TardisMcContext *ctx) { return ctx ? ctx->sw.last_sweep_skip : -1; }
 int tardis_mc_last_table_offsets(TardisMcContext *ctx) { return ctx ? ctx->last_table_offsets : -1; }
 int tardis_mc_last_compactions(TardisMcContext *ctx) { return ctx ? ctx->wv.compactions : -1; }
 int tardis_mc_last_tracker_defer(TardisMcContext *ctx) { return ctx ? ctx->wv.last_tracker_defer : -1; }
diff --git a/tardis_amd/csrc/tau_prefix.hpp b/tardis_amd/csrc/tau_prefix.hpp
--- a/tardis_amd/csrc/tau_prefix.hpp
+++ b/tardis_amd/csrc/tau_prefix.hpp
@@ -19,12 +19,12 @@
 }
 
 __global__ void __launch_bounds__(256) tau_prefix_kernel(const double *__restrict__ tau_t, int n_lines, double *__restrict__ pfx,
-                                                         double *__restrict__ rowsum, int *__restrict__ negative)
+                                                         double *__restrict__ rowsum, int *__restrict__ negative, int step = 1, int offset = 0)
 {
     __shared__ DD part[256];
     const int s = blockIdx.x, tid = threadIdx.x;
     const double *__restrict__ row = tau_t + (size_t)s * (size_t)n_lines;
-    double *__restrict__ out = pfx + (size_t)s * (size_t)(n_lines + 1);
+    double *__restrict__ out = pfx + (size_t)s * (size_t)(n_lines + 1) * (size_t)step + (size_t)offset;
     const int per = (n_lines + 255) / 256;
     const int i0 = min(tid * per, n_lines), i1 = min(i0 + per, n_lines);
     DD acc = {0.0, 0.0};
@@ -48,10 +48,10 @@
     __syncthreads();
     acc = part[tid];
     for (int i = i0; i < i1; ++i) {
-        out[i] = acc.hi + acc.lo;
+        out[(size_t)i * (size_t)step] = acc.hi + acc.lo;
         dd_add(acc, row[i]);
     }
-    if (i1 == n_lines && i0 < n_lines) out[n_lines] = acc.hi + acc.lo;
+    if (i1 == n_lines && i0 < n_lines) out[(size_t)n_lines * (size_t)step] = acc.hi + acc.lo;
     if (n_lines == 0 && tid == 0) out[0] = 0.0;
     if (neg) atomicOr(negative, 1);
 }
diff --git a/tardis_amd/engine.py b/tardis_amd/engine.py
--- a/tardis_amd/engine.py
+++ b/tardis_amd/engine.py
@@ -364,6 +364,9 @@
 
     def last_variant(self) -> int:
         return int(self._L.tardis_mc_last_variant(self._h))
+
+    def last_sweep_skip(self) -> int:
+        return int(self._L.tardis_mc_last_sweep_skip(self._h))
 
     def last_table_offsets(self) -> int:
         return int(self._L.tardis_mc_last_table_offsets(self._h))
```

After: 41.25 million packets/s (median of 6 runs). +9.4%, better.
